# StarsX/RayTracedGGX

Measured on AMD Instinct MI355X. Metric: Mrays/s + ms/frame, bunny 1920x1080 1spp+denoise, 1/2/4/8 GPUs, higher is better.
Workload: dtype f32; 1 GPU; configs[1]: bunny.obj + rnl_cross env, 1920x1080, 1spp GGX reflection + full denoise chain (refl H,V; diff H,V, shared-memory variant; temporal; tone map), all-metal default materials, dt=1/60; parallelism=row strips x1, history_apron_rows=18, history_overreach_rows=0, setup_priming_frames=256, trace_workgroup_waves=12

## Files before the change

include/rtggx.h:

```cpp
#ifndef RTGGX_H
#define RTGGX_H

#include <stddef.h>
#include <stdint.h>

#ifdef __cplusplus
extern "C" {
#endif

typedef struct rtggx_context rtggx_context;

enum { RTGGX_GROUND = 0, RTGGX_MODEL_OBJ = 1, RTGGX_NUM_MESH = 2 };

typedef struct RtggxCBGlobal {
  float    WorldViewProjs[2][16];
  float    WorldViewProjsPrev[2][16];
  float    Worlds[2][12];
  float    WorldITs0[12];
  float    WorldIT1[11];
  uint32_t FrameIndex;
} RtggxCBGlobal;
typedef struct RtggxRayGenConstants {
  float ProjToWorld[16];
  float EyePt[4];
// ... 61 lines not shown
int  rtggx_create(rtggx_context** out, uint32_t width, uint32_t height, int device);
void rtggx_destroy(rtggx_context* ctx);

int  rtggx_set_strip(rtggx_context* ctx, uint32_t row_begin, uint32_t row_end);

int  rtggx_set_history_apron(rtggx_context* ctx, uint32_t rows);
int  rtggx_history_overreach(rtggx_context* ctx, uint32_t* rows, int reset);

int  rtggx_set_stream(rtggx_context* ctx, void* hip_stream);
int  rtggx_get_stream(rtggx_context* ctx, void** hip_stream);
#define RTGGX_MAX_PEERS 16
#define RTGGX_IPC_HANDLE_BYTES 64
int  rtggx_set_history_peers(rtggx_context* ctx, uint32_t world, const uint32_t* bounds, void* const* tss0, void* const* tss1);
int  rtggx_history_ipc_export(rtggx_context* ctx, void* handles, size_t bytes);
int  rtggx_history_ipc_open(rtggx_context* ctx, const void* handles, size_t bytes, void** tss0, void** tss1);

int  rtggx_set_async_compute(rtggx_context* ctx, int enable);

int  rtggx_set_mesh(rtggx_context* ctx, uint32_t slot, const float* verts, uint32_t num_verts,
                    const uint32_t* indices, uint32_t num_indices);
int  rtggx_set_env(rtggx_context* ctx, int format, uint32_t size, uint32_t mips, const void* data, size_t bytes);
enum { RTGGX_ENV_EQUIRECT = 0, RTGGX_ENV_VCROSS = 1, RTGGX_ENV_HCROSS = 2 };
enum { RTGGX_PIXELS_RGBE8 = 0, RTGGX_PIXELS_RGB32F = 1 };
int  rtggx_set_env_image(rtggx_context* ctx, int layout, int pixels, uint32_t width, uint32_t height, const void* data, size_t bytes,
                         uint32_t cube_size);
int  rtggx_generate_env_mips(rtggx_context* ctx);
#define RTGGX_ENV_FILTER_MIN_SAMPLES 64u
#define RTGGX_ENV_FILTER_MAX_SAMPLES 4096u
int  rtggx_prefilter_env(rtggx_context* ctx, uint32_t samples);
int  rtggx_set_material(rtggx_context* ctx, uint32_t mesh, const float base_color[4], float roughness, float metallic);
int  rtggx_set_metallic(rtggx_context* ctx, uint32_t mesh, float metallic);
int  rtggx_set_sampler(rtggx_context* ctx, int vndf);
int  rtggx_set_ray_rate(rtggx_context* ctx, uint32_t pixels_per_ray);
#define RTGGX_MAX_RECURSION_DEPTH 4u
int  rtggx_set_max_recursion_depth(rtggx_context* ctx, uint32_t depth);
#define RTGGX_MAX_SAMPLES_PER_PIXEL 8u
int  rtggx_set_samples_per_pixel(rtggx_context* ctx, uint32_t samples);
#define RTGGX_MIN_SAMPLE_SET 256u
#define RTGGX_MAX_SAMPLE_SET 65536u
int  rtggx_set_sample_set(rtggx_context* ctx, uint32_t size);
int  rtggx_set_accumulation(rtggx_context* ctx, int enable);
int  rtggx_reset_accumulation(rtggx_context* ctx);
int  rtggx_accumulated_frames(rtggx_context* ctx, uint32_t* frames);
int  rtggx_present_accumulation(rtggx_context* ctx);

typedef struct RtggxScore {
  uint64_t index;
  uint32_t frame_index;
  uint32_t pad;
  uint64_t pixels, covered;
  uint64_t skipped_out, skipped_raw;
  double se_out_rgb, se_out_luma;
  double se_raw_rgb, se_raw_luma;
  double ref_rgb2, ref_luma2;
  double se_out_rgb_cov, se_raw_rgb_cov, ref_rgb2_cov;
} RtggxScore;
enum { RTGGX_SCORE_RING = 256 };
int  rtggx_set_reference(rtggx_context* ctx, const void* rgba16f, size_t bytes);
int  rtggx_reference_from_accumulation(rtggx_context* ctx);
int  rtggx_set_scoring(rtggx_context* ctx, int enable);
int  rtggx_read_scores(rtggx_context* ctx, RtggxScore* out, uint32_t capacity, uint32_t* count);

int  rtggx_set_sample_map(rtggx_context* ctx, const uint8_t* counts, uint32_t blocks_x, uint32_t blocks_y);
int  rtggx_read_sample_map(rtggx_context* ctx, uint8_t* counts, uint32_t capacity, uint32_t* blocks_x, uint32_t* blocks_y);

int  rtggx_build_as(rtggx_context* ctx);

int  rtggx_refit_as(rtggx_context* ctx, uint32_t slot, const float* verts, uint32_t num_verts);
int  rtggx_refit_as_device(rtggx_context* ctx, uint32_t slot, const float* device_verts, uint32_t num_verts, void* hip_stream);
int  rtggx_set_refit_policy(rtggx_context* ctx, float rebuild_ratio, uint32_t steps_per_frame);
int  rtggx_refit_stats(rtggx_context* ctx, uint32_t slot, float* cost_ratio, uint32_t* refits, uint32_t* rebuilds);

int  rtggx_update_frame(rtggx_context* ctx, const RtggxFrameConstants* constants);
int  rtggx_update_as(rtggx_context* ctx);
int  rtggx_transform_sh(rtggx_context* ctx);
int  rtggx_render_visibility(rtggx_context* ctx);
int  rtggx_ray_trace(rtggx_context* ctx);
int  rtggx_denoise(rtggx_context* ctx, int use_shared_mem);
int  rtggx_tone_map(rtggx_context* ctx);

int  rtggx_debug_fuse_tone_map(rtggx_context* ctx, int mode);
int  rtggx_debug_placement(rtggx_context* ctx, int force_small, uint32_t* key, uint32_t* where);
int  rtggx_debug_tile_words(rtggx_context* ctx, int enable);
int  rtggx_debug_static_sky(rtggx_context* ctx, int enable);
int  rtggx_debug_sky_runs(rtggx_context* ctx, uint32_t* runs, uint32_t capacity, uint32_t* tiles_x, uint32_t* tiles_y, uint32_t* threshold);
int  rtggx_debug_settled_sky(rtggx_context* ctx, int enable);
int  rtggx_debug_settled_words(rtggx_context* ctx, uint32_t* words0, uint32_t* words1, uint32_t capacity, uint32_t* blocks_x, uint32_t* blocks_y, uint32_t* epoch);
int  rtggx_debug_collapse_weights(rtggx_context* ctx, const float* set, float* get);
int  rtggx_debug_fence_wait(rtggx_context* ctx, double* us_total, uint32_t* waits, int reset);

int  rtggx_sync(rtggx_context* ctx);
int  rtggx_ray_count(rtggx_context* ctx, uint64_t* rays);
int  rtggx_ray_total(rtggx_context* ctx, uint64_t* rays, int reset);
int  rtggx_debug_counters(rtggx_context* ctx, uint32_t* out, uint32_t n, int reset);
int  rtggx_debug_trace_split(rtggx_context* ctx, uint32_t work_per_wave, uint32_t max_shift, int capacity, uint32_t* last_demand);
int  rtggx_debug_trace_residency(rtggx_context* ctx, uint32_t force_waves, uint32_t* waves, float* share);
int  rtggx_debug_environment(rtggx_context* ctx, const float* dirs3, const float* levels, uint32_t n, int level0_path, float* rgb3);
int  rtggx_get_timings(rtggx_context* ctx, RtggxTimings* out);
#define RTGGX_KERNEL_RING 4096
int  rtggx_enable_timing(rtggx_context* ctx, int mode);
int  rtggx_kernel_times(rtggx_context* ctx, float* ms, uint32_t capacity, uint32_t* count);

int  rtggx_debug_shader_clock(rtggx_context* ctx, double* mhz);

int  rtggx_copy_bandwidth(rtggx_context* ctx, size_t bytes, int iterations, double* gbytes_per_s);

int  rtggx_buffer_size(rtggx_context* ctx, int buffer_id, size_t* bytes);
int  rtggx_readback(rtggx_context* ctx, int buffer_id, void* dst, size_t bytes);
int  rtggx_buffer_ptr(rtggx_context* ctx, int buffer_id, void** device_ptr);
int  rtggx_upload(rtggx_context* ctx, int buffer_id, const void* src, size_t bytes);
int  rtggx_frame_parity(rtggx_context* ctx, uint32_t* parity);
int  rtggx_bvh_root(rtggx_context* ctx, uint32_t slot, int32_t* root);

int  rtggx_trace_rays(rtggx_context* ctx, const float* rays, uint32_t n, float* out);

int  rtggx_trace_occlusion(rtggx_context* ctx, const float* rays, uint32_t n, uint32_t* occluded);

int  rtggx_set_sun(rtggx_context* ctx, const float direction[3], const float irradiance[3]);

int  rtggx_set_sun_reflections(rtggx_context* ctx, int enable);

#define RTGGX_MAX_SUN_ANGLE_DEGREES 10.0f
int  rtggx_set_sun_angle(rtggx_context* ctx, float degrees);

typedef struct RtggxLight {
  float position[3];  float range;
  float intensity[3]; float radius;
  float axis[3];      float cos_outer;
  float cos_inner;    float pad[3];
} RtggxLight;
#define RTGGX_MAX_LIGHTS 8u
int  rtggx_set_lights(rtggx_context* ctx, const RtggxLight* lights, uint32_t count);

int  rtggx_set_light_reflections(rtggx_context* ctx, int enable);

int  rtggx_set_light_sampling(rtggx_context* ctx, int mode);

typedef struct RtggxSunEstimate {
  double cos2_cone, cos2_ring;
  double peak_luma, mean_luma;
  double weight_all, weight_cone, weight_ring;
  double ring_rgb[3];
  double background[3];
  double excess[3];
  double moment[3];
  float  background_half[3];
  float  direction[3], irradiance[3];
  uint32_t found, removed;
  uint32_t peak_face, peak_x, peak_y;
  uint32_t texels_cone, texels_ring, texels_lit;
  uint32_t pad;
} RtggxSunEstimate;
int  rtggx_sun_from_env(rtggx_context* ctx, float cone_degrees, float ring_degrees, float min_contrast, int remove, RtggxSunEstimate* out);

#ifdef __cplusplus
}
#endif
#endif
```

raytracedggx_amd/capi.py:

```python
import ctypes as C
import os

import numpy as np

_HERE = os.path.dirname(os.path.abspath(__file__))
LIB_PATH = os.path.join(_HERE, "librtggx.so")

BUF_VISIBILITY, BUF_DEPTH, BUF_NORMAL, BUF_ROUGH_METAL, BUF_VELOCITY, BUF_RT_REFL, BUF_RT_DIFF, BUF_TSS0, BUF_TSS1, \
    BUF_FLT_RFL, BUF_FLT_DFF, BUF_BACKBUFFER, BUF_SH_COEFFS, BUF_BVH_NODES0, BUF_BVH_TRIS0, BUF_BVH_NODES1, BUF_BVH_TRIS1, \
    BUF_TLAS, BUF_ENV, BUF_BVH4_NODES0, BUF_BVH4_NODES1, BUF_BIN_WORK, BUF_BVH4_TOP0, BUF_BVH4_TOP1, BUF_EXCHANGE_TOKENS, \
    BUF_ACC_REFL, BUF_ACC_DIFF, BUF_CONVERGED = range(28)
MAX_PEERS, IPC_HANDLE_BYTES = 16, 64
FORMAT_RGBA32F, FORMAT_RGBA16F, FORMAT_BC6H_UF16, FORMAT_BC6H_SF16 = 2, 10, 95, 96
ENV_EQUIRECT, ENV_VCROSS, ENV_HCROSS = 0, 1, 2
PIXELS_RGBE8, PIXELS_RGB32F = 0, 1
ENV_FILTER_MIN_SAMPLES, ENV_FILTER_MAX_SAMPLES = 64, 4096
MAX_SUN_ANGLE_DEGREES = 10.0
MAX_LIGHTS = 8

_BUF_DTYPE = {BUF_VISIBILITY: np.uint32, BUF_DEPTH: np.uint32, BUF_NORMAL: np.uint32, BUF_ROUGH_METAL: np.uint16,
              BUF_VELOCITY: np.uint32, BUF_RT_REFL: np.uint32, BUF_RT_DIFF: np.uint32, BUF_TSS0: np.uint64, BUF_TSS1: np.uint64,
              BUF_FLT_RFL: np.uint64, BUF_FLT_DFF: np.uint64, BUF_BACKBUFFER: np.uint32, BUF_SH_COEFFS: np.float32,
              BUF_BVH_NODES0: np.uint32, BUF_BVH_TRIS0: np.uint32, BUF_BVH_NODES1: np.uint32, BUF_BVH_TRIS1: np.uint32,
              BUF_TLAS: np.float32, BUF_ENV: np.uint16, BUF_BVH4_NODES0: np.uint32, BUF_BVH4_NODES1: np.uint32, BUF_BIN_WORK: np.uint32,
              BUF_BVH4_TOP0: np.uint32, BUF_BVH4_TOP1: np.uint32, BUF_EXCHANGE_TOKENS: np.uint32,
              BUF_ACC_REFL: np.float32, BUF_ACC_DIFF: np.float32, BUF_CONVERGED: np.uint64}

EXPORTS = ["rtggx_last_error", "rtggx_create", "rtggx_destroy", "rtggx_set_strip", "rtggx_set_stream", "rtggx_set_mesh",
           "rtggx_set_env", "rtggx_set_material", "rtggx_set_metallic", "rtggx_build_as", "rtggx_update_frame", "rtggx_update_as",
           "rtggx_transform_sh", "rtggx_render_visibility", "rtggx_ray_trace", "rtggx_denoise", "rtggx_tone_map", "rtggx_sync",
           "rtggx_ray_count", "rtggx_get_timings", "rtggx_enable_timing", "rtggx_buffer_size", "rtggx_readback", "rtggx_buffer_ptr",
           "rtggx_upload", "rtggx_frame_parity", "rtggx_bvh_root", "rtggx_trace_rays", "rtggx_ray_total", "rtggx_kernel_times", "rtggx_debug_counters", "rtggx_debug_trace_split", "rtggx_debug_trace_residency", "rtggx_get_stream", "rtggx_set_history_peers", "rtggx_history_ipc_export", "rtggx_history_ipc_open",
           "rtggx_set_async_compute", "rtggx_set_history_apron", "rtggx_history_overreach", "rtggx_copy_bandwidth", "rtggx_refit_as", "rtggx_refit_as_device", "rtggx_refit_stats", "rtggx_set_refit_policy", "rtggx_set_sampler", "rtggx_set_ray_rate", "rtggx_set_max_recursion_depth", "rtggx_set_samples_per_pixel", "rtggx_debug_fuse_tone_map", "rtggx_debug_placement", "rtggx_debug_tile_words", "rtggx_debug_static_sky", "rtggx_debug_settled_sky", "rtggx_debug_settled_words", "rtggx_debug_sky_runs", "rtggx_debug_collapse_weights", "rtggx_debug_fence_wait", "rtggx_debug_shader_clock", "rtggx_debug_environment",
           "rtggx_set_accumulation", "rtggx_reset_accumulation", "rtggx_accumulated_frames", "rtggx_present_accumulation", "rtggx_set_sample_set",
           "rtggx_set_reference", "rtggx_reference_from_accumulation", "rtggx_set_scoring", "rtggx_read_scores",
           "rtggx_set_env_image", "rtggx_generate_env_mips", "rtggx_prefilter_env",
           "rtggx_set_sample_map", "rtggx_read_sample_map", "rtggx_trace_occlusion", "rtggx_set_sun", "rtggx_set_sun_reflections",
           "rtggx_sun_from_env", "rtggx_set_sun_angle", "rtggx_set_lights", "rtggx_set_light_reflections", "rtggx_set_light_sampling"]
SCORE_RING = 256


class Timings(C.Structure):
    _fields_ = [(n, C.c_float) for n in ("update_as", "visibility", "ray_trace", "spatial_refl_h", "spatial_refl_v",
                                         "spatial_diff_h", "spatial_diff_v", "temporal", "tone_map", "frame", "ray_trace_kernel")]


class Score(C.Structure):
    _fields_ = [("index", C.c_uint64), ("frame_index", C.c_uint32), ("pad", C.c_uint32), ("pixels", C.c_uint64), ("covered", C.c_uint64),
                ("skipped_out", C.c_uint64), ("skipped_raw", C.c_uint64)] + \
               [(n, C.c_double) for n in ("se_out_rgb", "se_out_luma", "se_raw_rgb", "se_raw_luma", "ref_rgb2", "ref_luma2",
                                          "se_out_rgb_cov", "se_raw_rgb_cov", "ref_rgb2_cov")]

    def as_dict(self):
        return {n: getattr(self, n) for n, _ in self._fields_ if n != "pad"}


class SunEstimate(C.Structure):
    _fields_ = [(n, C.c_double) for n in ("cos2_cone", "cos2_ring", "peak_luma", "mean_luma", "weight_all", "weight_cone", "weight_ring")] + \
               [(n, C.c_double * 3) for n in ("ring_rgb", "background", "excess", "moment")] + \
               [(n, C.c_float * 3) for n in ("background_half", "direction", "irradiance")] + \
               [(n, C.c_uint32) for n in ("found", "removed", "peak_face", "peak_x", "peak_y", "texels_cone", "texels_ring", "texels_lit", "pad")]

    def as_dict(self):
        out = {"bytes": bytes(self)}
        for n, t in self._fields_:
            if n != "pad":
                v = getattr(self, n)
                out[n] = v if t in (C.c_double, C.c_uint32) else np.array(list(v), np.float64 if t == C.c_double * 3 else np.float32)
        return out


class Light(C.Structure):
    _fields_ = [("position", C.c_float * 3), ("range", C.c_float), ("intensity", C.c_float * 3), ("radius", C.c_float),
                ("axis", C.c_float * 3), ("cos_outer", C.c_float), ("cos_inner", C.c_float), ("pad", C.c_float * 3)]

    @classmethod
    def of(cls, position, intensity, range, radius=0.0, axis=(0.0, 0.0, 0.0), cos_outer=-1.0, cos_inner=1.0):
        return cls((C.c_float * 3)(*position), range, (C.c_float * 3)(*intensity), radius, (C.c_float * 3)(*axis), cos_outer, cos_inner)


_lib = None


def load():
    global _lib
    if _lib is not None:
        return _lib
    if not os.path.exists(LIB_PATH):
        raise ImportError("librtggx.so is not built: run `python -c 'import __graft_entry__ as g; g.build()'` "
                          "or `make -C raytracedggx_amd` (hipcc, gfx950). There is no CPU path.")
    L = C.CDLL(LIB_PATH)
    L.rtggx_last_error.restype = C.c_char_p
    vp = C.c_void_p
    L.rtggx_create.argtypes = [C.POINTER(vp), C.c_uint32, C.c_uint32, C.c_int]
    L.rtggx_destroy.argtypes = [vp]
    L.rtggx_destroy.restype = None
    L.rtggx_set_strip.argtypes = [vp, C.c_uint32, C.c_uint32]
    L.rtggx_set_stream.argtypes = [vp, vp]
    L.rtggx_set_async_compute.argtypes = [vp, C.c_int]
    L.rtggx_set_ray_rate.argtypes = [vp, C.c_uint32]
    L.rtggx_set_max_recursion_depth.argtypes = [vp, C.c_uint32]
    L.rtggx_set_samples_per_pixel.argtypes = [vp, C.c_uint32]
    L.rtggx_set_sample_set.argtypes = [vp, C.c_uint32]
    L.rtggx_set_accumulation.argtypes = [vp, C.c_int]
    L.rtggx_reset_accumulation.argtypes = [vp]
    L.rtggx_accumulated_frames.argtypes = [vp, C.POINTER(C.c_uint32)]
    L.rtggx_present_accumulation.argtypes = [vp]
    L.rtggx_set_reference.argtypes = [vp, vp, C.c_size_t]
    L.rtggx_reference_from_accumulation.argtypes = [vp]
    L.rtggx_set_scoring.argtypes = [vp, C.c_int]
    L.rtggx_read_scores.argtypes = [vp, C.POINTER(Score), C.c_uint32, C.POINTER(C.c_uint32)]
    L.rtggx_set_sample_map.argtypes = [vp, vp, C.c_uint32, C.c_uint32]
    L.rtggx_read_sample_map.argtypes = [vp, vp, C.c_uint32, C.POINTER(C.c_uint32), C.POINTER(C.c_uint32)]
    L.rtggx_set_history_apron.argtypes = [vp, C.c_uint32]
    L.rtggx_debug_shader_clock.argtypes = [vp, C.POINTER(C.c_double)]
    L.rtggx_refit_as.argtypes = [vp, C.c_uint32, vp, C.c_uint32]
# ... 41 lines not shown
    pass


def _p(a):
    return a.ctypes.data_as(C.c_void_p)


class Context:

    def __init__(self, width, height, device=0):
        self.L = load()
        self.W, self.H = int(width), int(height)
        h = C.c_void_p()
        self._check(self.L.rtggx_create(C.byref(h), self.W, self.H, int(device)))
        self.h = h

    def _check(self, rc):
        if rc != 0:
            raise RtggxError("librtggx: %s (code %d)" % (self.L.rtggx_last_error().decode(), rc))

    def close(self):
        if getattr(self, "h", None):
            self.L.rtggx_destroy(self.h)
            self.h = None

    def __del__(self):
        try:
            self.close()
        except Exception:
            pass

    def set_strip(self, row_begin, row_end):
        self._check(self.L.rtggx_set_strip(self.h, row_begin, row_end))

    def set_stream(self, stream_handle):
        self._check(self.L.rtggx_set_stream(self.h, C.c_void_p(stream_handle)))

    def shader_clock_mhz(self):
        m = C.c_double()
        self._check(self.L.rtggx_debug_shader_clock(self.h, C.byref(m)))
        return m.value

    def copy_bandwidth(self, nbytes=1 << 30, iterations=8):
        g = C.c_double()
        self._check(self.L.rtggx_copy_bandwidth(self.h, int(nbytes), int(iterations), C.byref(g)))
        return g.value

    def set_history_apron(self, rows):
        self._check(self.L.rtggx_set_history_apron(self.h, int(rows)))

    def history_overreach(self, reset=True):
        n = C.c_uint32()
        self._check(self.L.rtggx_history_overreach(self.h, C.byref(n), int(reset)))
        return n.value

    def set_async_compute(self, enable):
        self._check(self.L.rtggx_set_async_compute(self.h, int(bool(enable))))

    def set_mesh(self, slot, verts, indices):
        v = np.ascontiguousarray(verts, np.float32).reshape(-1, 6)
        i = np.ascontiguousarray(indices, np.uint32).reshape(-1)
        self._check(self.L.rtggx_set_mesh(self.h, slot, _p(v), v.shape[0], _p(i), i.size))

    def refit_as(self, slot, verts):
        v = np.ascontiguousarray(verts, np.float32).reshape(-1, 6)
        self._check(self.L.rtggx_refit_as(self.h, slot, _p(v), v.shape[0]))

    def refit_as_device(self, slot, device_ptr, num_verts, stream=0):
        self.L.rtggx_refit_as_device.argtypes = [C.c_void_p, C.c_uint32, C.c_void_p, C.c_uint32, C.c_void_p]
        self._check(self.L.rtggx_refit_as_device(self.h, slot, C.c_void_p(int(device_ptr)), int(num_verts), C.c_void_p(int(stream) or None)))

    def fence_wait(self, reset=True):
        us, n = C.c_double(0.0), C.c_uint32(0)
        self.L.rtggx_debug_fence_wait.argtypes = [C.c_void_p, C.POINTER(C.c_double), C.POINTER(C.c_uint32), C.c_int]
        self._check(self.L.rtggx_debug_fence_wait(self.h, C.byref(us), C.byref(n), 1 if reset else 0))
        return us.value, n.value

    def fuse_tone_map(self, mode):
        self._check(self.L.rtggx_debug_fuse_tone_map(self.h, -1 if mode is None else 1 if mode else 0))

    def tile_words(self, enable):
        self._check(self.L.rtggx_debug_tile_words(self.h, 1 if enable else 0))

    def static_sky(self, enable):
        self._check(self.L.rtggx_debug_static_sky(self.h, 1 if enable else 0))

    def sky_runs(self):
        tiles = ((self.W + 15) // 16) * ((self.H + 15) // 16 + 1)
        runs = np.zeros(tiles, np.uint32)
        tx, ty, th = C.c_uint32(), C.c_uint32(), C.c_uint32()
        self.L.rtggx_debug_sky_runs.argtypes = [C.c_void_p, C.c_void_p, C.c_uint32, C.c_void_p, C.c_void_p, C.c_void_p]
        self._check(self.L.rtggx_debug_sky_runs(self.h, _p(runs), tiles, C.byref(tx), C.byref(ty), C.byref(th)))
        return runs[:tx.value * ty.value].reshape(ty.value, tx.value), int(th.value)

    def settled_sky(self, enable):
        self.L.rtggx_debug_settled_sky.argtypes = [C.c_void_p, C.c_int]
        self._check(self.L.rtggx_debug_settled_sky(self.h, 1 if enable else 0))

    def settled_words(self):
        n = ((self.W + 63) // 64) * ((self.H + 3) // 4)
        w = np.zeros((2, n), np.uint32)
        bx, by, ep = C.c_uint32(), C.c_uint32(), C.c_uint32()
        self.L.rtggx_debug_settled_words.argtypes = [C.c_void_p, C.c_void_p, C.c_void_p, C.c_uint32, C.c_void_p, C.c_void_p, C.c_void_p]
        self._check(self.L.rtggx_debug_settled_words(self.h, _p(w[0]), _p(w[1]), n, C.byref(bx), C.byref(by), C.byref(ep)))
        return np.ascontiguousarray(w.reshape(2, bx.value, by.value).transpose(0, 2, 1)), int(ep.value)

    def placement(self, force_small=-1):
        k, w = C.c_uint32(), C.c_uint32()
        self.L.rtggx_debug_placement.argtypes = [C.c_void_p, C.c_int, C.c_void_p, C.c_void_p]
        self._check(self.L.rtggx_debug_placement(self.h, int(force_small), C.byref(k), C.byref(w)))
        names = ("main", "B", "C", "R", "?")
        key = {n: bool((k.value >> i) & 1) for i, n in enumerate(("small", "strip", "deforming", "diffuse", "caller_stream"))}
        where = {"raster": names[(w.value >> 16) & 15], "gen": names[w.value & 15], "trace": names[(w.value >> 4) & 15], "shade": names[(w.value >> 8) & 15], "frames_in_flight": (w.value >> 12) & 15}
        return key, where

    def collapse_weights(self, area=None, tris=None):
        self.L.rtggx_debug_collapse_weights.argtypes = [C.c_void_p, C.c_void_p, C.c_void_p]
        get = (C.c_float * 2)()
        if area is not None:
            st = (C.c_float * 2)(float(area), float(tris))
            self._check(self.L.rtggx_debug_collapse_weights(self.h, st, get))
        else:
            self._check(self.L.rtggx_debug_collapse_weights(self.h, None, get))
        return float(get[0]), float(get[1])

    def set_history_peers(self, bounds, tss0, tss1):
        self.L.rtggx_set_history_peers.argtypes = [C.c_void_p, C.c_uint32, C.c_void_p, C.c_void_p, C.c_void_p]
        if bounds is None:
            self._check(self.L.rtggx_set_history_peers(self.h, 0, None, None, None))
            return
        world = len(bounds) - 1
        b = (C.c_uint32 * (world + 1))(*[int(x) for x in bounds])
        p0 = (C.c_void_p * world)(*[C.c_void_p(int(x) or None) for x in tss0])
        p1 = (C.c_void_p * world)(*[C.c_void_p(int(x) or None) for x in tss1])
        self._check(self.L.rtggx_set_history_peers(self.h, world, b, p0, p1))

    def history_ipc_export(self):
        self.L.rtggx_history_ipc_export.argtypes = [C.c_void_p, C.c_void_p, C.c_size_t]
        buf = C.create_string_buffer(2 * IPC_HANDLE_BYTES)
        self._check(self.L.rtggx_history_ipc_export(self.h, buf, len(buf.raw)))
        return bytes(buf.raw)

    def history_ipc_open(self, handles):
        self.L.rtggx_history_ipc_open.argtypes = [C.c_void_p, C.c_char_p, C.c_size_t, C.c_void_p, C.c_void_p]
        p0, p1 = C.c_void_p(), C.c_void_p()
        self._check(self.L.rtggx_history_ipc_open(self.h, bytes(handles), len(handles), C.byref(p0), C.byref(p1)))
        return int(p0.value), int(p1.value)

    def set_sampler(self, vndf):
        self._check(self.L.rtggx_set_sampler(self.h, 1 if vndf else 0))

    def set_ray_rate(self, pixels_per_ray):
        self._check(self.L.rtggx_set_ray_rate(self.h, int(pixels_per_ray)))

    def set_max_recursion_depth(self, depth):
        self._check(self.L.rtggx_set_max_recursion_depth(self.h, int(depth)))

    def set_samples_per_pixel(self, samples):
        self._check(self.L.rtggx_set_samples_per_pixel(self.h, int(samples)))

    def set_sample_set(self, size):
        self._check(self.L.rtggx_set_sample_set(self.h, int(size)))

    def set_accumulation(self, enable):
        self._check(self.L.rtggx_set_accumulation(self.h, 1 if enable else 0))

# ... 261 lines not shown
```

raytracedggx_amd/csrc/debug.hip:

```cpp
#include <cstring>
#include "capi_internal.h"
#include "rt_queue.h"
namespace rt {
__global__ void __launch_bounds__(256) copyKernel(const float4* __restrict__ src, float4* __restrict__ dst, size_t n) {
  for (size_t i = (size_t)blockIdx.x * 256u + threadIdx.x; i < n; i += (size_t)gridDim.x * 256u) dst[i] = src[i];
}
typedef float __attribute__((ext_vector_type(4))) CopyVec4;
__global__ void __launch_bounds__(256) copyKernelNT(const CopyVec4* __restrict__ src, CopyVec4* __restrict__ dst, size_t n) {
  for (size_t i = (size_t)blockIdx.x * 256u + threadIdx.x; i < n; i += (size_t)gridDim.x * 256u) __builtin_nontemporal_store(__builtin_nontemporal_load(&src[i]), &dst[i]);
}
}
using namespace rt;

extern "C" {
int rtggx_ray_count(rtggx_context* c, uint64_t* rays) {
  RT_CHECK_CTX(c);
  uint32_t h[256];
  RT_HIP(syncStreams(c));
  RT_HIP(hipMemcpy(h, c->lastRayCounter32, sizeof h, hipMemcpyDeviceToHost));
  uint64_t s = 0; for (auto v : h) s += v;
  *rays = s;
  return 0;
}

int rtggx_debug_counters(rtggx_context* c, uint32_t* out, uint32_t n, int reset) {
  RT_CHECK_CTX(c);
  if (n > 768) { setError("rtggx_debug_counters: at most 768 words"); return -1; }
  RT_HIP(syncStreams(c));
  RT_HIP(hipMemcpy(out, c->rayCounterBuf + 1024, (size_t)n * 4, hipMemcpyDeviceToHost));
  if (reset) { RT_HIP(hipMemset(c->rayCounterBuf + 1024, 0, 768 * 4)); RT_HIP(hipStreamSynchronize(nullptr)); }
  return 0;
}

int rtggx_debug_fence_wait(rtggx_context* c, double* usTotal, uint32_t* waits, int reset) {
  RT_CHECK_CTX(c);
  if (usTotal) *usTotal = c->fenceWaitUs;
  if (waits) *waits = c->fenceWaits;
  if (reset) { c->fenceWaitUs = 0.0; c->fenceWaits = 0u; }
  return 0;
}
int rtggx_debug_fuse_tone_map(rtggx_context* c, int mode) {
  RT_CHECK_CTX(c);
  c->fuseToneMap = mode < 0 ? -1 : mode != 0;
  return 0;
}
int rtggx_debug_tile_words(rtggx_context* c, int enable) {
  RT_CHECK_CTX(c);
  c->useTileWords = enable != 0;
  c->sky.breakRuns(SkyBreak::TileWordsSwitch);
  return 0;
}
int rtggx_debug_static_sky(rtggx_context* c, int enable) {
  RT_CHECK_CTX(c);
  c->sky.enableStaticSky(enable != 0);
  return 0;
}
int rtggx_debug_sky_runs(rtggx_context* c, uint32_t* runs, uint32_t capacity, uint32_t* tilesX, uint32_t* tilesY, uint32_t* threshold) {
  RT_CHECK_CTX(c);
  const uint32_t n = c->sky.genTilesX() * c->sky.genTilesY();
  if (!runs || capacity < n || n > c->skyTiles) { setError("rtggx_debug_sky_runs: room for %u words", n); return -1; }
  RT_HIP(syncStreams(c));
  if (n) RT_HIP(hipMemcpy(runs, c->cur().skyRun, (size_t)n * 4, hipMemcpyDeviceToHost));
  for (uint32_t i = 0; i < n; ++i) runs[i] = (runs[i] >> 8) == c->sky.epoch() ? runs[i] & 0xFFu : 0u;
  if (tilesX) *tilesX = c->sky.genTilesX();
  if (tilesY) *tilesY = c->sky.genTilesY();
  if (threshold) *threshold = RT_SKY_PREV_RUN + 1u;
  return 0;
}
int rtggx_debug_settled_sky(rtggx_context* c, int enable) {
  RT_CHECK_CTX(c);
  c->sky.enableSettledSky(enable != 0);
  return 0;
}
int rtggx_debug_settled_words(rtggx_context* c, uint32_t* words0, uint32_t* words1, uint32_t capacity, uint32_t* blocksX, uint32_t* blocksY, uint32_t* epoch) {
  RT_CHECK_CTX(c);
  const uint32_t n = c->settledX * c->settledY;
  if (!words0 || !words1 || capacity < n) { setError("rtggx_debug_settled_words: room for %u words each", n); return -1; }
  RT_HIP(syncStreams(c));
  uint32_t* const out[2] = {words0, words1};
  for (int p = 0; p < 2 && n; ++p)
    RT_HIP(hipMemcpy2D(out[p], (size_t)c->settledY * 4, c->settled[p] + c->settledPitch + 1u, (size_t)c->settledPitch * 4, (size_t)c->settledY * 4, c->settledX, hipMemcpyDeviceToHost));
  if (blocksX) *blocksX = c->settledX;
  if (blocksY) *blocksY = c->settledY;
  if (epoch) *epoch = c->sky.epoch();
  return 0;
}
int rtggx_debug_placement(rtggx_context* c, int forceSmall, uint32_t* key, uint32_t* where) {
  RT_CHECK_CTX(c);
  if (forceSmall < -1 || forceSmall > 1) { setError("rtggx_debug_placement: force_small is -1, 0 or 1"); return -1; }
  c->forcePlacement = forceSmall;
  if (forceSmall >= 0) c->lastTraceSmall = forceSmall == 1;
  if (key) *key = c->lastPlacement[0];
  if (where) *where = c->lastPlacement[1];
  return 0;
}
int rtggx_debug_collapse_weights(rtggx_context* c, const float* set, float* get) {
  RT_CHECK_CTX(c);
  if (set) { if (!(set[0] >= 0.0f) || !(set[1] >= 0.0f) || !(set[0] + set[1] > 0.0f)) { setError("rtggx_debug_collapse_weights: two non-negative weights, not both zero"); return -1; }
             c->collapseWeights[0] = set[0]; c->collapseWeights[1] = set[1]; }
  if (get) { get[0] = c->collapseWeights[0]; get[1] = c->collapseWeights[1]; }
  return 0;
}
int rtggx_debug_trace_residency(rtggx_context* c, uint32_t forceWaves, uint32_t* waves, float* share) {
  RT_CHECK_CTX(c);
  if (forceWaves != 0u && forceWaves != 10u && forceWaves != 12u && forceWaves != 14u && forceWaves != 16u) { setError("rtggx_debug_trace_residency: %u waves: 0, 10, 12, 14 or 16", forceWaves); return -1; }
  c->traceWavesForced = forceWaves;
  if (forceWaves) c->traceWaves = forceWaves;
  if (waves) *waves = c->traceWaves;
  if (share) *share = c->traceShare;
  return 0;
}

int rtggx_debug_environment(rtggx_context* c, const float* dirs3, const float* levels, uint32_t n, int level0Path, float* rgb3) {
  RT_CHECK_CTX(c);
  if (!c->env.texels) { setError("rtggx_debug_environment: no environment map"); return -1; }
  if (n == 0 || !dirs3 || !rgb3 || (!levels && !level0Path)) { setError("rtggx_debug_environment: no directions, levels or result (n %u)", n); return -1; }
  DevBuf<float> dD, dL, dO;
  hipError_t e = alloc(dD, (size_t)n * 3);
  if (e == hipSuccess) e = alloc(dO, (size_t)n * 3);
  if (e == hipSuccess && levels) e = alloc(dL, (size_t)n);
  if (e == hipSuccess) e = hipMemcpy(dD, dirs3, (size_t)n * 12, hipMemcpyHostToDevice);
  if (e == hipSuccess && levels) e = hipMemcpy(dL, levels, (size_t)n * 4, hipMemcpyHostToDevice);
  int r = 0;
  if (e == hipSuccess) r = launchDebugEnvironment(c, dD, dL, n, level0Path, dO, c->streamMain);
  if (e == hipSuccess && !r) e = hipStreamSynchronize(c->streamMain);
  if (e == hipSuccess && !r) e = hipMemcpy(rgb3, dO, (size_t)n * 12, hipMemcpyDeviceToHost);
  if (e != hipSuccess) { setError("rtggx_debug_environment: %s", hipGetErrorString(e)); return -2; }
  return r;
}

int rtggx_debug_trace_split(rtggx_context* c, uint32_t workPerWave, uint32_t maxShift, int capacity, uint32_t* lastDemand) {
  RT_CHECK_CTX(c);
// ... 245 lines not shown
```

raytracedggx_amd/csrc/denoise.hip:

```cpp
#include <cstring>
#include <type_traits>
#include "rtggx_context.h"

namespace rt {

#define RT_RADIUS 16
#ifndef RT_VBW
#define RT_VBW 16
#define RT_VBH 16
#endif

RT_DEV float rcpFast(float x) { return __builtin_amdgcn_rcpf(x); }

struct GTexel { float nx, ny, nz, nw, rough, metal, depth; };

RT_DEV GTexel loadG(const uint32_t* __restrict__ normal, const uint16_t* __restrict__ roughMetal, const uint32_t* __restrict__ depth32,
                    int x, int y, int W, int H) {
  GTexel g;
  if (x < 0 || y < 0 || x >= W || y >= H) { g.nx = g.ny = g.nz = -1023.0f; g.nw = 0.0f; g.rough = 0.0f; g.metal = 0.0f; g.depth = 0.0f; return g; }
  const size_t i = (size_t)y * W + x;
  const uint32_t n = normal[i];
  g.nx = (float)(2 * (int)(n & 1023u) - 1023);
  g.ny = (float)(2 * (int)((n >> 10) & 1023u) - 1023);
  g.nz = (float)(2 * (int)((n >> 20) & 1023u) - 1023);
// ... 35 lines not shown
RT_DEV uint32_t skyRunMin6(const uint32_t* words, uint32_t epoch, uint32_t i0, uint32_t i1, uint32_t i2, uint32_t i3, uint32_t i4, uint32_t i5) {
  uint32_t w[6];
  asm volatile("s_load_dword %0, %6, %7\n\ts_load_dword %1, %6, %8\n\ts_load_dword %2, %6, %9\n\ts_load_dword %3, %6, %10\n\ts_load_dword %4, %6, %11\n\ts_load_dword %5, %6, %12\n\ts_waitcnt lgkmcnt(0)"
               : "=&s"(w[0]), "=&s"(w[1]), "=&s"(w[2]), "=&s"(w[3]), "=&s"(w[4]), "=&s"(w[5])
               : "s"(words), "s"(RT_SGPR(i0 * 4u)), "s"(RT_SGPR(i1 * 4u)), "s"(RT_SGPR(i2 * 4u)), "s"(RT_SGPR(i3 * 4u)), "s"(RT_SGPR(i4 * 4u)), "s"(RT_SGPR(i5 * 4u)) : "memory");
  uint32_t run = 0xFFu;
#pragma unroll
  for (int k = 0; k < 6; ++k) run = min(run, (w[k] >> 8) == epoch ? w[k] & 0xFFu : 0u);
  return run;
}

typedef uint32_t U2 __attribute__((ext_vector_type(2)));
typedef uint32_t U4 __attribute__((ext_vector_type(4)));
RT_DEV void loadTemporalWords(const uint32_t* rowA, const uint32_t* rowB, const uint32_t* col0, const uint32_t* col1, const uint32_t* col2,
                              U4& a4, U2& a2, U4& b4, U2& b2, U4& c0, U4& c1, U4& c2) {
  asm volatile("s_load_dwordx4 %0, %7, 0x0\n\ts_load_dwordx2 %1, %7, 0x10\n\ts_load_dwordx4 %2, %8, 0x0\n\ts_load_dwordx2 %3, %8, 0x10\n\t"
               "s_load_dwordx4 %4, %9, 0x0\n\ts_load_dwordx4 %5, %10, 0x0\n\ts_load_dwordx4 %6, %11, 0x0\n\ts_waitcnt lgkmcnt(0)"
               : "=&s"(a4), "=&s"(a2), "=&s"(b4), "=&s"(b2), "=&s"(c0), "=&s"(c1), "=&s"(c2)
               : "s"(rowA), "s"(rowB), "s"(col0), "s"(col1), "s"(col2) : "memory");
}
RT_DEV void loadToneMapWords(const uint32_t* col0, const uint32_t* col1, const uint32_t* col2, U4& a4, U2& a2, U4& b4, U2& b2, U4& c4, U2& c2) {
  asm volatile("s_load_dwordx4 %0, %6, 0x0\n\ts_load_dwordx2 %1, %6, 0x10\n\ts_load_dwordx4 %2, %7, 0x0\n\ts_load_dwordx2 %3, %7, 0x10\n\t"
               "s_load_dwordx4 %4, %8, 0x0\n\ts_load_dwordx2 %5, %8, 0x10\n\ts_waitcnt lgkmcnt(0)"
               : "=&s"(a4), "=&s"(a2), "=&s"(b4), "=&s"(b2), "=&s"(c4), "=&s"(c2) : "s"(col0), "s"(col1), "s"(col2) : "memory");
}

#define RT_LOG2E 1.44269504088896341f

struct Centre { float nx, ny, nz, depth, rough, gaussK , depthK ; };
#define RT_NORMAL_SCALE_SQ 1046529.0f
RT_DEV float log2OfDot(float I) {
  const float d = fmaxf((I - RT_NORMAL_SCALE_SQ) * (1.0f / RT_NORMAL_SCALE_SQ), -1.0f);
  const float xr = 1.0f + d;
  const float dropped = (1.0f - xr) + d;
  return __builtin_fmaf(dropped, RT_LOG2E, __builtin_amdgcn_logf(xr));
}
template <bool DIFFUSE, int UNIFORM = 0>
RT_DEV float tapWeight(const Centre& c, int i, float nx, float ny, float nz, float depth, float rough) {
#pragma clang fp contract(fast)
  const float I = __builtin_fmaf(c.nz, nz, __builtin_fmaf(c.ny, ny, c.nx * nx));
  const float lg = log2OfDot(I);
  const float dd = fabsf(c.depth - depth) * c.depthK;
  if (DIFFUSE) return __builtin_amdgcn_exp2f(__builtin_fmaf(32.0f, lg, -dd));
  const float pw = 512.0f * lg;
  const float e = __builtin_fmaf(c.gaussK, (float)(i * i), -dd);
  const float w = __builtin_amdgcn_exp2f(pw >= 128.0f ? pw : pw + e);
  if (UNIFORM == 2) return w;
  const float flag = (__float_as_uint(rough) >> 31) ? 0.0f : 1.0f;
  if (UNIFORM == 1) return w * flag;
  const float t = saturatef(fabsf(fabsf(rough) - c.rough) * 2.0f);
  return (w * (1.0f - t * t * (3.0f - 2.0f * t))) * flag;
}
template <bool DIFFUSE>
RT_DEV Centre makeCentre(float nx, float ny, float nz, float depth, float rough, int W, int H) {
  Centre c; c.nx = nx; c.ny = ny; c.nz = nz; c.depth = depth; c.rough = rough;
  const int br = DIFFUSE ? 0 : (int)clampf(0.1f * rough * (float)W, 0.0f, (float)H * 0.05f);
  const float sigma = (float)(br + 1) * (1.0f / 3.0f);
  c.gaussK = (-0.5f * RT_LOG2E) * rcpFast(sigma * sigma);
  c.depthK = depth * (4.0f * RT_LOG2E);
  return c;
}
template <int MODE>
RT_DEV void storeFiltered(const Targets& T, size_t pix, float mx, float my, float mz, float wsum) {
  const float rw = rcpFast(wsum);
  f3 mu = mk3(mx * rw, my * rw, mz * rw);
  if (MODE == 0 || MODE == 2) T.scratch[pix] = packRGBA16F(mu.x, mu.y, mu.z, 0.0f);
  if (MODE == 1) { mu = ITM3(mu); const uint2 v = packRGBA16F(mu.x, mu.y, mu.z, 1.0f); if (T.fltRfl) T.fltRfl[pix] = v; T.fltDff[pix] = v; }
  if (MODE == 3) {
    const f4 dest = unpackRGBA16F(T.fltRfl[pix]);
    mu = ITM3(mu);
    T.fltDff[pix] = packRGBA16F(dest.x + mu.x, dest.y + mu.y, dest.z + mu.z, dest.w);
  }
}
template <int MODE>
RT_DEV void storeSkipped(const Targets& T, size_t pix) {
  if (MODE == 1) { const f3 s = unpackR11G11B10F(T.rtRefl[pix]); const uint2 v = packRGBA16F(s.x, s.y, s.z, 0.0f); if (T.fltRfl) T.fltRfl[pix] = v; T.fltDff[pix] = v; }
}
template <int MODE>
RT_DEV f3 tapColour(const Targets& T, size_t ti) {
  if (MODE & 1) { const f4 v = unpackRGBA16F(T.scratch[ti]); return mk3(v.x, v.y, v.z); }
  return TM3(unpackR11G11B10F(MODE >= 2 ? T.rtDiff[ti] : T.rtRefl[ti]));
}

template <int MODE>
__global__ void __launch_bounds__(256) spatialDirectKernel(Targets T) {
  constexpr bool vertical = (MODE & 1) != 0;
  constexpr bool diffuse = MODE >= 2;
  const int x = blockIdx.x * 64 + (threadIdx.x & 63);
  const int y = T.rowBegin + blockIdx.y * 4 + (threadIdx.x >> 6);
  if (x >= T.W || y >= T.rowEnd) return;
  const size_t pix = (size_t)y * T.W + x;
  const GTexel gc = loadG(T.normal, T.roughMetal, T.depth32, x, y, T.W, T.H);
  if (diffuse ? (gc.nw <= 0.0f || gc.metal >= 1.0f) : (gc.nw <= 0.0f)) { storeSkipped<MODE>(T, pix); return; }
  const Centre c = makeCentre<diffuse>(gc.nx, gc.ny, gc.nz, gc.depth, gc.rough, T.W, T.H);
  float mx = 0.0f, my = 0.0f, mz = 0.0f, wsum = 0.0f;
  for (int i = -RT_RADIUS; i <= RT_RADIUS; ++i) {
    const int tx = vertical ? x : x + i, ty = vertical ? y + i : y;
    const bool inside = tx >= 0 && ty >= 0 && tx < T.W && ty < T.H;
    const GTexel g = loadG(T.normal, T.roughMetal, T.depth32, tx, ty, T.W, T.H);
    if (diffuse && (g.nw <= 0.0f || g.metal >= 1.0f)) continue;
    const f3 src = inside ? tapColour<MODE>(T, (size_t)ty * T.W + tx) : mk3(0.0f, 0.0f, 0.0f);
    const float w = tapWeight<diffuse>(c, i, g.nx, g.ny, g.nz, g.depth, g.nw > 0.0f ? g.rough : __uint_as_float(__float_as_uint(g.rough) | 0x80000000u));
    mx = __builtin_fmaf(src.x, w, mx); my = __builtin_fmaf(src.y, w, my); mz = __builtin_fmaf(src.z, w, mz);
    wsum += w;
  }
  storeFiltered<MODE>(T, pix, mx, my, mz, wsum);
}

typedef float V4 __attribute__((ext_vector_type(4)));
template <int MODE>
__global__ void __launch_bounds__(256) spatialTiledKernel(Targets T) {
  constexpr bool vertical = (MODE & 1) != 0;
  constexpr bool diffuse = MODE >= 2;
  constexpr int BW = vertical ? RT_VBW : 64, BH = vertical ? RT_VBH : 4;
  constexpr int TW = vertical ? RT_VBW : 96, TH = vertical ? RT_VBH + 2 * RT_RADIUS : 4;
  constexpr int PER = vertical ? BW * BH / 256 : 1, ROWSTEP = 256 / BW;
  constexpr int N = TW * TH;
  __shared__ V4 smA[N], smB[N];
  __shared__ uint32_t roughLo, roughHi, unflagged;
  if (threadIdx.x == 0) { roughLo = 0xFFFFFFFFu; roughHi = 0u; unflagged = 0u; }
  const int bx0 = blockIdx.x * BW, by0 = T.rowBegin + blockIdx.y * BH;
  const int lx = threadIdx.x % BW, ly = threadIdx.x / BW;
  const int x = bx0 + lx;

  static_assert(RT_VBW <= 32 && RT_VBH <= 32, "the V block spans at most two tiles across and three down");
  bool nothingDrawn;
  { const uint32_t txLast = (uint32_t)T.tilesX - 1u, tx0 = (uint32_t)bx0 >> 4, tx1 = min(tx0 + 1u, txLast);
    const uint32_t ty0 = (uint32_t)(by0 - T.tileRow0) >> 4, ty1 = (uint32_t)(min(by0 + BH, T.rowEnd) - 1 - T.tileRow0) >> 4;
    const uint32_t r0 = ty0 * (uint32_t)T.tilesX, r1 = ty1 * (uint32_t)T.tilesX, rm = ((ty0 + ty1) >> 1) * (uint32_t)T.tilesX;
    if (MODE == 1 && T.skyRun != nullptr && skyRunMin6(T.skyRun, T.skyEpoch, r0 + tx0, r0 + tx1, rm + tx0, rm + tx1, r1 + tx0, r1 + tx1) >= RT_SKY_V_RUN) return;
    nothingDrawn = vertical ? tileWordsOr6(T.tileWords, r0 + tx0, r0 + tx1, rm + tx0, rm + tx1, r1 + tx0, r1 + tx1) == 0u
                            : tileWordsOr(T.tileWords, r0 + tx0, r0 + tx1, r0 + min(tx0 + 2u, txLast), r0 + min(tx0 + 3u, txLast)) == 0u; }
  if (nothingDrawn) {
    if (MODE == 1) {
#pragma unroll
      for (int k = 0; k < PER; ++k) { const int y = by0 + ly + k * ROWSTEP; if (x < T.W && y < T.rowEnd) storeSkipped<MODE>(T, (size_t)y * T.W + x); }
    }
    return;
  }
  bool todo[PER]; bool any = false;
#pragma unroll
  for (int k = 0; k < PER; ++k) {
    const int y = by0 + ly + k * ROWSTEP;
    todo[k] = false;
    if (x < T.W && y < T.rowEnd) {
      const size_t pix = (size_t)y * T.W + x;
      const bool skip = (T.normal[pix] >> 30) == 0u || (diffuse && (T.roughMetal[pix] >> 8) == 255u);
      if (skip) storeSkipped<MODE>(T, pix); else { todo[k] = true; any = true; }
    }
  }
  if (!__syncthreads_or(any ? 1 : 0)) return;

  const int ox = vertical ? bx0 : bx0 - RT_RADIUS, oy = vertical ? by0 - RT_RADIUS : by0;
  uint32_t myLo = 0xFFFFFFFFu, myHi = 0u, myUnflagged = 0u;
  for (int t = threadIdx.x; t < N; t += 256) {
    const int tx = ox + t % TW, ty = oy + t / TW;
    float v[8] = {0.0f, 0.0f, 0.0f, 0.0f, 0.0f, 0.0f, 0.0f, 0.0f};
    const bool inside = tx >= 0 && ty >= 0 && tx < T.W && ty < T.H;
    const GTexel g = loadG(T.normal, T.roughMetal, T.depth32, tx, ty, T.W, T.H);
    v[3] = g.depth; v[4] = g.rough;
    if (diffuse) {
      if (g.nw > 0.0f && g.metal < 1.0f) {
        const f3 src = tapColour<MODE>(T, (size_t)ty * T.W + tx);
        v[0] = g.nx; v[1] = g.ny; v[2] = g.nz; v[5] = src.x; v[6] = src.y; v[7] = src.z;
      }
    } else {
      v[0] = g.nx; v[1] = g.ny; v[2] = g.nz;
      if (g.nw <= 0.0f) { v[4] = __uint_as_float(__float_as_uint(g.rough) | 0x80000000u); myUnflagged = 1u; }
      else { myLo = min(myLo, __float_as_uint(g.rough)); myHi = max(myHi, __float_as_uint(g.rough)); }
      if (inside) { const f3 src = tapColour<MODE>(T, (size_t)ty * T.W + tx); v[5] = src.x; v[6] = src.y; v[7] = src.z; }
    }
    smA[t] = V4{v[0], v[1], v[2], v[3]}; smB[t] = V4{v[4], v[5], v[6], v[7]};
  }
  if (!diffuse) {
    for (int o = 32; o > 0; o >>= 1) { myLo = min(myLo, (uint32_t)__shfl_down((int)myLo, o)); myHi = max(myHi, (uint32_t)__shfl_down((int)myHi, o)); }
    const unsigned long long anyUnflagged = __ballot(myUnflagged != 0u);
    if ((threadIdx.x & 63) == 0) { atomicMin(&roughLo, myLo); atomicMax(&roughHi, myHi); if (anyUnflagged) atomicOr(&unflagged, 1u); }
  }
  __syncthreads();
  const int uniform = diffuse ? 0 : (roughLo != roughHi ? 0 : unflagged ? 1 : 2);

  auto filter = [&](auto uniformTag) {
    constexpr int UNIFORM = decltype(uniformTag)::value;
#pragma unroll
    for (int k = 0; k < PER; ++k) {
      if (!todo[k]) continue;
      const int y = by0 + ly + k * ROWSTEP;
      const int ci = vertical ? (ly + k * ROWSTEP + RT_RADIUS) * TW + lx : ly * TW + lx + RT_RADIUS;
      const V4 ca = smA[ci];
      const Centre c = makeCentre<diffuse>(ca.x, ca.y, ca.z, ca.w, smB[ci].x, T.W, T.H);
      float mx = 0.0f, my = 0.0f, mz = 0.0f, wsum = 0.0f;
      typedef __attribute__((address_space(3))) const V4 LdsV4;
      LdsV4* pa = (LdsV4*)&smA[ci - RT_RADIUS * (vertical ? TW : 1)]; LdsV4* pb = (LdsV4*)&smB[ci - RT_RADIUS * (vertical ? TW : 1)];
      asm volatile("" : "+v"(pa)); asm volatile("" : "+v"(pb));
#pragma unroll
      for (int i = -RT_RADIUS; i <= RT_RADIUS; ++i) {
        const int ti = (i + RT_RADIUS) * (vertical ? TW : 1);
        const V4 a = pa[ti], b = pb[ti];
        const float w = tapWeight<diffuse, UNIFORM>(c, i, a.x, a.y, a.z, a.w, b.x);
        mx = __builtin_fmaf(b.y, w, mx); my = __builtin_fmaf(b.z, w, my); mz = __builtin_fmaf(b.w, w, mz);
        wsum += w;
      }
      storeFiltered<MODE>(T, (size_t)y * T.W + x, mx, my, mz, wsum);
    }
// ... 296 lines not shown
  if (WORDS && T.settledIn != nullptr) {
    static_assert(RT_TM_ROWS == 4 * RT_TP_ROWS, "a tone-map block is four blocks of the temporal pass high");
    const uint32_t* col = T.settledIn + blockIdx.x * T.settledPitch + blockIdx.y * 4u;
    U4 a4, b4, c4; U2 a2, b2, c2;
    loadToneMapWords(col, col + T.settledPitch, col + 2u * T.settledPitch, a4, a2, b4, b2, c4, c2);
    const uint32_t w[18] = {a4.x, a4.y, a4.z, a4.w, a2.x, a2.y, b4.x, b4.y, b4.z, b4.w, b2.x, b2.y, c4.x, c4.y, c4.z, c4.w, c2.x, c2.y};
    bool skip = true;
#pragma unroll
    for (int k = 0; k < 18; ++k) skip = skip & settledWord(w[k], T.skyEpoch);
    if (skip) return;
  }
  {
    const int ox = blockIdx.x * 64 - 1, oy = T.rowBegin + blockIdx.y * RT_TM_ROWS - 1;
    constexpr int N = (RT_TM_ROWS + 2) * 66, PER = (N + 255) / 256;
    f4 c[PER];
#pragma unroll
    for (int k = 0; k < PER; ++k) { const int t = threadIdx.x + 256 * k; c[k] = t < N ? loadRGBA16(T.scratch, ox + t % 66, oy + t / 66, W, H) : f4{0.0f, 0.0f, 0.0f, 0.0f}; }
#pragma unroll
    for (int k = 0; k < PER; ++k) {
      const int t = threadIdx.x + 256 * k;
      if (t < N) tile[t / 66][t % 66] = make_float4(c[k].x * rcpFast(c[k].x + 0.5f), c[k].y * rcpFast(c[k].y + 0.5f), c[k].z * rcpFast(c[k].z + 0.5f), c[k].w);
    }
  }
  __syncthreads();
  const int lx = (threadIdx.x & 63) + 1;
  const int x = blockIdx.x * 64 + (threadIdx.x & 63);
  if (x >= T.W) return;
#pragma unroll
  for (int k = 0; k < RT_TM_ROWS / 4; ++k) {
    const int ly = (threadIdx.x >> 6) + 4 * k + 1;
    const int y = T.rowBegin + blockIdx.y * RT_TM_ROWS + (threadIdx.x >> 6) + 4 * k;
    if (y >= T.rowEnd) continue;
    const float4 c0 = tile[ly][lx], c1 = tile[ly][lx - 1], c2 = tile[ly][lx + 1], c3 = tile[ly - 1][lx], c4 = tile[ly + 1][lx];
    float lx_ = -4.0f * c0.x, ly_ = -4.0f * c0.y, lz_ = -4.0f * c0.z;
    lx_ += c1.x; ly_ += c1.y; lz_ += c1.z;
    lx_ += c2.x; ly_ += c2.y; lz_ += c2.z;
    lx_ += c3.x; ly_ += c3.y; lz_ += c3.z;
    lx_ += c4.x; ly_ += c4.y; lz_ += c4.z;
    T.backbuffer[(size_t)y * W + x] = packRGBA8(c0.x - 0.2f * lx_, c0.y - 0.2f * ly_, c0.z - 0.2f * lz_, c0.w);
  }
}

static Targets makeTargets(rtggx_context* c, const FrameParams& fp, RowPass pass) {
  Targets T;
  const InputSet& set = c->cur();
  T.normal = set.normal; T.roughMetal = set.roughMetal; T.depth32 = set.depth32; T.velocity = set.velocity;
  T.rtRefl = set.rtRefl; T.rtDiff = set.rtDiff;
  T.scratch = c->tss[c->frameParity]; T.history = c->tss[c->frameParity ^ 1u]; T.fltRfl = c->fltRfl; T.fltDff = c->fltDff; T.backbuffer = c->backbuffer;
  T.W = (int)fp.W; T.H = (int)fp.H;
  uint32_t rb, re; passRows(fp, pass, rb, re);
  T.rowBegin = (int)rb; T.rowEnd = (int)re;
  passRows(fp, ROWS_FINAL, rb, re);
  T.outBegin = (int)rb; T.outEnd = (int)re;
  const bool strip = fp.rowBegin > 0u || fp.rowEnd < fp.H;
  T.histLo = (int)(fp.rowBegin > c->historyApron ? fp.rowBegin - c->historyApron : 0u);
  T.histHi = (int)(fp.rowEnd + c->historyApron < fp.H ? fp.rowEnd + c->historyApron : fp.H);
  T.histReach = strip ? c->histReach : nullptr;
  const bool peers = strip && c->peerWorld > 1u && c->dPeerTable != nullptr;
  T.peerHist = peers ? reinterpret_cast<const uint2* const*>(c->dPeerTable.get()) + (c->frameParity ^ 1u) * RT_MAX_PEERS : nullptr;
  T.peerBounds = peers ? reinterpret_cast<const uint32_t*>(reinterpret_cast<const uint2* const*>(c->dPeerTable.get()) + 2 * RT_MAX_PEERS) : nullptr;
  T.peerWorld = peers ? (int)c->peerWorld : 0;
  { uint32_t gb, ge; passRows(fp, ROWS_GBUFFER, gb, ge);
    T.tileWords = c->tileWords(gb, ge); T.tilesX = (int)((fp.W + 15) / 16); T.tileRow0 = (int)gb; }
  T.skyRun = nullptr; T.skyEpoch = 0u;
  T.settledOut = nullptr; T.settledIn = nullptr; T.settledPitch = c->settledPitch;
  return T;
}

static bool wholeFrame(const rtggx_context* c, const FrameParams& fp) { return fp.rowBegin == 0u && fp.rowEnd == fp.H && fp.W == c->W && fp.H == c->H; }

int launchDenoise(rtggx_context* c, const FrameParams& fp, int useLds, hipStream_t s, hipEvent_t done, bool fuseToneMap) {
  c->frameParity ^= 1u;
  if (fp.rowEnd <= fp.rowBegin) return 0;
  const Targets TH = makeTargets(c, fp, ROWS_GBUFFER), TV = makeTargets(c, fp, ROWS_VFILTER), TT = makeTargets(c, fp, ROWS_TEMPORAL);
  const dim3 block(256);
  auto grid = [&](const Targets& T, uint32_t bw, uint32_t bh) { return dim3((fp.W + bw - 1) / bw, (T.rowEnd - T.rowBegin + bh - 1) / bh); };
  auto mark = [&](int i) { if (c->timing) hipEventRecord(c->tev[i], s); };
  const bool anyDiffuse = fp.mat.RoughMetals[0][1] < 1.0f || fp.mat.RoughMetals[1][1] < 1.0f;
  c->fltRflIsFltDff = !anyDiffuse;
  Targets TVr = TV; if (!anyDiffuse) TVr.fltRfl = nullptr;
  { SkyChain::VFacts now;
    now.frame = c->frameCounter; now.gbufferRow0 = (uint32_t)TV.tileRow0; now.rows[0] = (uint32_t)TV.rowBegin; now.rows[1] = (uint32_t)TV.rowEnd; now.fltRflNull = TVr.fltRfl == nullptr;
    if (c->sky.reflectionV(now) && useLds) { TVr.skyRun = c->cur().skyRun; TVr.skyEpoch = c->sky.epoch(); } }
  if (useLds) {
    hipLaunchKernelGGL(spatialTiledKernel<0>, grid(TH, 64, 4), block, 0, s, TH); mark(4);
    hipLaunchKernelGGL(spatialTiledKernel<1>, grid(TV, RT_VBW, RT_VBH), block, 0, s, TVr); mark(5);
    if (anyDiffuse) hipLaunchKernelGGL(spatialTiledKernel<2>, grid(TH, 64, 4), block, 0, s, TH);
    mark(6);
    if (anyDiffuse) hipLaunchKernelGGL(spatialTiledKernel<3>, grid(TV, RT_VBW, RT_VBH), block, 0, s, TV);
    mark(7);
  } else if (!anyDiffuse) {
    hipLaunchKernelGGL(spatialDirectKernel<0>, grid(TH, 64, 4), block, 0, s, TH); mark(4);
    hipLaunchKernelGGL(spatialDirectKernel<1>, grid(TV, 64, 4), block, 0, s, TVr); mark(5); mark(6); mark(7);
  } else {
    hipLaunchKernelGGL(spatialDirectKernel<0>, grid(TH, 64, 4), block, 0, s, TH); mark(4);
    hipLaunchKernelGGL(spatialDirectKernel<1>, grid(TV, 64, 4), block, 0, s, TV); mark(5);
    hipLaunchKernelGGL(spatialDirectKernel<2>, grid(TH, 64, 4), block, 0, s, TH); mark(6);
    hipLaunchKernelGGL(spatialDirectKernel<3>, grid(TV, 64, 4), block, 0, s, TV); mark(7);
  }
  Targets TTs = TT;
  { SkyChain::TemporalFacts now;
    now.frame = c->frameCounter; now.gbufferRow0 = (uint32_t)TT.tileRow0; now.rows[0] = (uint32_t)TT.rowBegin; now.rows[1] = (uint32_t)TT.rowEnd;
    now.parity = c->frameParity; now.width = fp.W; now.fused = fuseToneMap; now.whole = wholeFrame(c, fp);
    const SkyChain::TemporalDecision d = c->sky.temporal(now);
    if (d.keepsWords) { TTs.settledOut = c->settled[c->frameParity]; TTs.skyEpoch = c->sky.epoch(); }
    if (d.maySkip) { TTs.settledIn = c->settled[c->frameParity ^ 1u]; TTs.skyRun = c->cur().skyRun; } }
  if (fuseToneMap) {
    const dim3 g((fp.W + RT_TT_W - 1) / RT_TT_W, (uint32_t)(TT.outEnd - TT.outBegin + RT_TT_H - 1) / RT_TT_H), b(RT_TT_TW * RT_TT_TH);
    launch(temporalToneKernel, g, b, s, nullptr, done, TT);
    c->sky.backBufferWrittenElsewhere();
  } else launch(TTs.settledOut ? temporalKernel<true> : temporalKernel<false>, grid(TT, 64, RT_TP_ROWS), block, s, nullptr, done, TTs);
  mark(8);
  RT_HIP(hipGetLastError());
  return 0;
}

int launchToneMap(rtggx_context* c, const FrameParams& fp, hipStream_t s, hipEvent_t done, const uint2* source) {
  if (fp.rowEnd <= fp.rowBegin) return 0;
  Targets T = makeTargets(c, fp, ROWS_FINAL);
  if (source) T.scratch = const_cast<uint2*>(source);
  { SkyChain::ToneMapFacts now;
    now.frame = c->frameCounter; now.rows[0] = (uint32_t)T.rowBegin; now.rows[1] = (uint32_t)T.rowEnd; now.parity = c->frameParity; now.fromTss = source == nullptr; now.whole = wholeFrame(c, fp);
    if (c->sky.toneMap(now)) { T.settledIn = c->settled[c->frameParity]; T.skyEpoch = c->sky.epoch(); } }
  const dim3 grid((fp.W + 63) / 64, (uint32_t)(T.rowEnd - T.rowBegin + RT_TM_ROWS - 1) / RT_TM_ROWS), block(256);
  launch(T.settledIn ? toneMapKernel<true> : toneMapKernel<false>, grid, block, s, nullptr, done, T);
  RT_HIP(hipGetLastError());
  return 0;
}

}
```

raytracedggx_amd/csrc/frame.hip:

```cpp
#include <cstring>
#include <chrono>
#include "capi_internal.h"
#include "rt_queue.h"
namespace rt {
static void invert4x4(const float* a , float* out) {
  double m[16], inv[16];
  for (int i = 0; i < 16; ++i) m[i] = (double)a[i];
  inv[0] = m[5] * m[10] * m[15] - m[5] * m[11] * m[14] - m[9] * m[6] * m[15] + m[9] * m[7] * m[14] + m[13] * m[6] * m[11] - m[13] * m[7] * m[10];
  inv[4] = -m[4] * m[10] * m[15] + m[4] * m[11] * m[14] + m[8] * m[6] * m[15] - m[8] * m[7] * m[14] - m[12] * m[6] * m[11] + m[12] * m[7] * m[10];
  inv[8] = m[4] * m[9] * m[15] - m[4] * m[11] * m[13] - m[8] * m[5] * m[15] + m[8] * m[7] * m[13] + m[12] * m[5] * m[11] - m[12] * m[7] * m[9];
  inv[12] = -m[4] * m[9] * m[14] + m[4] * m[10] * m[13] + m[8] * m[5] * m[14] - m[8] * m[6] * m[13] - m[12] * m[5] * m[10] + m[12] * m[6] * m[9];
  inv[1] = -m[1] * m[10] * m[15] + m[1] * m[11] * m[14] + m[9] * m[2] * m[15] - m[9] * m[3] * m[14] - m[13] * m[2] * m[11] + m[13] * m[3] * m[10];
  inv[5] = m[0] * m[10] * m[15] - m[0] * m[11] * m[14] - m[8] * m[2] * m[15] + m[8] * m[3] * m[14] + m[12] * m[2] * m[11] - m[12] * m[3] * m[10];
  inv[9] = -m[0] * m[9] * m[15] + m[0] * m[11] * m[13] + m[8] * m[1] * m[15] - m[8] * m[3] * m[13] - m[12] * m[1] * m[11] + m[12] * m[3] * m[9];
  inv[13] = m[0] * m[9] * m[14] - m[0] * m[10] * m[13] - m[8] * m[1] * m[14] + m[8] * m[2] * m[13] + m[12] * m[1] * m[10] - m[12] * m[2] * m[9];
  inv[2] = m[1] * m[6] * m[15] - m[1] * m[7] * m[14] - m[5] * m[2] * m[15] + m[5] * m[3] * m[14] + m[13] * m[2] * m[7] - m[13] * m[3] * m[6];
  inv[6] = -m[0] * m[6] * m[15] + m[0] * m[7] * m[14] + m[4] * m[2] * m[15] - m[4] * m[3] * m[14] - m[12] * m[2] * m[7] + m[12] * m[3] * m[6];
  inv[10] = m[0] * m[5] * m[15] - m[0] * m[7] * m[13] - m[4] * m[1] * m[15] + m[4] * m[3] * m[13] + m[12] * m[1] * m[7] - m[12] * m[3] * m[5];
  inv[14] = -m[0] * m[5] * m[14] + m[0] * m[6] * m[13] + m[4] * m[1] * m[14] - m[4] * m[2] * m[13] - m[12] * m[1] * m[6] + m[12] * m[2] * m[5];
  inv[3] = -m[1] * m[6] * m[11] + m[1] * m[7] * m[10] + m[5] * m[2] * m[11] - m[5] * m[3] * m[10] - m[9] * m[2] * m[7] + m[9] * m[3] * m[6];
  inv[7] = m[0] * m[6] * m[11] - m[0] * m[7] * m[10] - m[4] * m[2] * m[11] + m[4] * m[3] * m[10] + m[8] * m[2] * m[7] - m[8] * m[3] * m[6];
  inv[11] = -m[0] * m[5] * m[11] + m[0] * m[7] * m[9] + m[4] * m[1] * m[11] - m[4] * m[3] * m[9] - m[8] * m[1] * m[7] + m[8] * m[3] * m[5];
  inv[15] = m[0] * m[5] * m[10] - m[0] * m[6] * m[9] - m[4] * m[1] * m[10] + m[4] * m[2] * m[9] + m[8] * m[1] * m[6] - m[8] * m[2] * m[5];
  const double det = m[0] * inv[0] + m[1] * inv[4] + m[2] * inv[8] + m[3] * inv[12];
// ... 73 lines not shown

int rtggx_transform_sh(rtggx_context* c) {
  RT_CHECK_CTX(c);
  return projectSH(c, c->streamAS);
}

struct Placement {
  bool small, strip, deforming, diffuse, callerStream;
  hipStream_t raster, gen, trace, shade;
  uint32_t framesInFlight;
  bool alternate, shadeWithTrace;
};
static Placement placeFrame(const rtggx_context* c, const FrameParams& fp, uint32_t frame) {
  Placement P;
  P.small = c->lastTraceSmall;
  P.strip = fp.rowBegin > 0u || fp.rowEnd < fp.H;
  P.deforming = c->mesh[0].deforming || c->mesh[1].deforming;
  P.diffuse = fp.mat.RoughMetals[0][1] < 1.0f || fp.mat.RoughMetals[1][1] < 1.0f;
  P.callerStream = c->externalStream;
  const bool async = c->asyncCompute && c->streamVis != nullptr;
  P.gen = async ? c->streamVis : c->streamMain;
  P.raster = P.gen;
  P.alternate = async && c->streamRefit != nullptr && P.small && !P.deforming && (frame & 1u) != 0u;
  P.trace = !async ? c->streamMain : P.alternate ? c->streamRefit : c->streamAS;
  P.shadeWithTrace = async && !c->timing && P.small && !P.deforming;
  P.shade = P.shadeWithTrace ? P.trace : c->streamMain;
  P.framesInFlight = async && !P.small && (P.deforming || P.diffuse) ? RT_SETS - 1u : RT_SETS;
  return P;
}

static int waitForSet(rtggx_context* c, const InputSet& set) {
  if (set.readRecorded && hipEventQuery(set.evRead) != hipSuccess) {
    const auto t0 = std::chrono::steady_clock::now();
    RT_HIP(hipEventSynchronize(set.evRead));
    c->fenceWaitUs += std::chrono::duration<double, std::micro>(std::chrono::steady_clock::now() - t0).count(); ++c->fenceWaits;
  }
  return 0;
}

int rtggx_render_visibility(rtggx_context* c) {
  RT_CHECK_CTX(c);
  if (!c->haveConstants) { setError("rtggx_render_visibility: no frame constants"); return -1; }
  if (!c->shDone && c->env.texels) { const int r = projectSH(c, c->streamAS); if (r) return r; }
  settleSetRead(c);
  ++c->frameCounter;
  c->maxDepth = c->depthRequested; c->samples = c->samplesRequested; c->accumulate = c->accumulateRequested; c->sun = c->sunRequested; c->sunAngle = c->sunAngleRequested; c->sunReflections = c->sunReflectionsRequested; c->lights = c->lightsRequested; c->lightReflections = c->lightReflectionsRequested; c->lightSampling = c->lightSamplingRequested;
  c->scoring = c->scoringRequested && c->reference != nullptr;
  c->sampleMap = c->sampleMapRequested;
  bool resendConstants = false;
  if (c->sampleSet != c->sampleSetRequested) {
    if (c->slotRendered) RT_HIP(syncStreams(c));
    c->sampleSet = c->sampleSetRequested;
    c->slots[c->slot].sampleMask = c->sampleSet - 1u;
    resendConstants = c->slotUploaded;
  }
  c->denoiseIssued = false; c->toneMapDone = false;
  c->selectSet(c->setAhead(1u));
  { const int r = waitForSet(c, c->cur()); if (r) return r; }
  const Placement P = placeFrame(c, c->slots[c->slot], c->frameCounter);
  if (P.framesInFlight < RT_SETS) { const int r = waitForSet(c, c->sets[c->setAhead(RT_SETS - P.framesInFlight)]); if (r) return r; }
  c->refitIssued = false;
  { const int r = issuePendingRefits(c, &c->refitIssued); if (r) return r; }
  const hipStream_t s = P.raster;
  if (c->evVisStream && c->evVisStream != s) RT_HIP(hipStreamWaitEvent(s, c->evVis, 0));
  { const FrameEvents& g = c->frameEvents(c->frameCounter + 2u);
    if (c->frameCounter >= 2u && g.genFrame == c->frameCounter - 2u && g.genStream != s) RT_HIP(hipStreamWaitEvent(s, g.gen, 0)); }
  if (c->slotUploaded && s != c->streamAS) RT_HIP(hipStreamWaitEvent(s, c->evAS, 0));
  if (c->refitIssued && c->asyncCompute && s != c->streamRefit) RT_HIP(hipStreamWaitEvent(s, c->evRefit, 0));
  if (c->timing) hipEventRecord(c->tev[2], s);
  int r = launchVisibility(c, c->slots[c->slot], s, c->streamVis ? c->evVis : nullptr);
  c->slotRendered = true;
  if (resendConstants) c->slotUploaded = false;
  if (c->streamVis) c->evVisStream = s;
  if (c->timing) hipEventRecord(c->tev[13], s);
  if (!r) r = issueRebuildSteps(c);
  return r;
}

int rtggx_ray_trace(rtggx_context* c) {
  RT_CHECK_CTX(c);
  if (!c->haveConstants || !c->asBuilt) { setError("rtggx_ray_trace: %s", c->asBuilt ? "no frame constants" : "rtggx_build_as has not been called"); return -1; }
  if (!c->env.texels) { setError("rtggx_ray_trace: no environment map"); return -1; }
  { const int r = ensureParams(c); if (r) return r; }
  const uint32_t f = c->frameCounter;
  const FrameParams& fp = c->slots[c->slot];
  const Placement P = placeFrame(c, fp, f);
  c->lastPlacement[0] = P.small | (P.strip << 1) | (P.deforming << 2) | (P.diffuse << 3) | (P.callerStream << 4);
  const auto streamId = [&](hipStream_t st) { return st == c->streamMain ? 0u : st == c->streamAS ? 1u : st == c->streamVis ? 2u : st == c->streamRefit ? 3u : 4u; };
  c->lastPlacement[1] = streamId(P.gen) | (streamId(P.trace) << 4) | (streamId(P.shade) << 8) | (P.framesInFlight << 12) | (streamId(P.raster) << 16);
  const hipStream_t sGen = P.gen;
  if (c->evVisStream && c->evVisStream != sGen) RT_HIP(hipStreamWaitEvent(sGen, c->evVis, 0));
  const hipStream_t sTrace = P.trace;
  c->traceSpillHalf = P.alternate ? 1u : 0u;
  if (sGen != sTrace) {
    if (c->frameEvents(f + 2u).traceRecorded) RT_HIP(hipStreamWaitEvent(sGen, c->frameEvents(f + 2u).trace, 0));
    if (c->slotUploaded) RT_HIP(hipStreamWaitEvent(sGen, c->evAS, 0));
  }
  if (c->refitIssued && c->asyncCompute) RT_HIP(hipStreamWaitEvent(sTrace, c->evRefit, 0));
  if (c->timing) hipEventRecord(c->tev[3], sGen);
  FrameEvents& ev = c->frameEvents(f);
  const bool shadeWithTrace = P.shadeWithTrace && sGen != sTrace && sTrace != c->streamMain;
  if (c->shadeWroteDiff && !P.diffuse && !c->lastFrameDiffuse && c->diffStream) {
    if (c->diffStream != sGen) { RT_HIP(hipEventRecord(c->evRT, c->diffStream)); RT_HIP(hipStreamWaitEvent(sGen, c->evRT, 0)); }
    c->shadeWroteDiff = false;
  }
  c->lastFrameDiffuse = P.diffuse;
  c->genCarriesDiff = !c->shadeWroteDiff;
  int r = launchRayTrace(c, fp, sGen, sTrace, shadeWithTrace ? nullptr : ev.trace);
  ev.traceRecorded = true;
  c->lastRayCounter32 = c->rayCounter32;
  c->shadeWroteDiff = !c->genCarriesDiff || P.diffuse;
  if (shadeWithTrace) {
    if (!c->genCarriesDiff && c->shadeStream && c->shadeStream != sTrace) {
      if (c->shadeStream == c->streamMain) { RT_HIP(hipEventRecord(c->evRT, c->streamMain)); RT_HIP(hipStreamWaitEvent(sTrace, c->evRT, 0)); }
      else if (c->frameEvents(f + 3u).traceRecorded) RT_HIP(hipStreamWaitEvent(sTrace, c->frameEvents(f + 3u).trace, 0));
    }
    if (!r) r = launchShade(c, fp, sTrace, ev.trace);
    c->shadeStream = sTrace;
    RT_HIP(hipStreamWaitEvent(c->streamMain, ev.trace, 0));
  } else {
    RT_HIP(hipStreamWaitEvent(c->streamMain, ev.trace, 0));
    if (!r) r = launchShade(c, fp, c->streamMain);
    c->shadeStream = c->streamMain;
  }
  c->diffStream = c->shadeStream;
  if (c->rayRate == 4u) {
    if (!r) r = launchReconstruct(c, fp, c->streamMain);
    c->diffStream = c->streamMain;
  }
  if (c->sun.on) {
    if (!r) r = launchSun(c, fp, c->streamMain);
    c->shadeStream = c->diffStream = c->streamMain;
  }
  if (c->lights.count) {
    if (!r) r = launchLights(c, fp, c->streamMain);
    c->shadeStream = c->diffStream = c->streamMain;
  }
  if (c->accumulate) {
    if (!r) r = launchAccumulate(c, fp, c->streamMain);
    if (!r) ++c->accumFrames;
  }
  c->setReadDeferred = (int)c->setIndex;
  if (c->timing) hipEventRecord(c->tev[14], c->streamMain);
  return r;
}

int rtggx_denoise(rtggx_context* c, int useSharedMem) {
  RT_CHECK_CTX(c);
  if (!c->haveConstants) { setError("rtggx_denoise: no frame constants"); return -1; }
  if (c->timing) hipEventRecord(c->tev[9], c->streamMain);
  const bool fuse = !c->timing && !c->scoring && (c->fuseToneMap > 0 || (c->fuseToneMap < 0 && c->lastTraceSmall));
  const int r = launchDenoise(c, c->slots[c->slot], useSharedMem, c->streamMain, fuse ? c->cur().evRead : nullptr, fuse);
  if (fuse) { c->cur().readRecorded = true; c->setReadDeferred = -1; } else c->setReadDeferred = (int)c->setIndex;
  if (!r && c->scoring && c->reference) { const int rs = launchScore(c, c->slots[c->slot], c->streamMain); if (rs) return rs; }
  c->denoiseIssued = true; c->toneMapDone = fuse && c->slots[c->slot].rowEnd > c->slots[c->slot].rowBegin;
  return r;
}

int rtggx_tone_map(rtggx_context* c) {
  RT_CHECK_CTX(c);
  if (!c->haveConstants) { setError("rtggx_tone_map: no frame constants"); return -1; }
  int r = 0;
  if (c->toneMapDone) c->toneMapDone = false;
  else {
    const bool carry = c->setReadDeferred >= 0;
    r = launchToneMap(c, c->slots[c->slot], c->streamMain, carry ? c->sets[c->setReadDeferred].evRead : nullptr);
// ... 15 lines not shown
```

raytracedggx_amd/csrc/raytrace.hip:

```cpp
#include <cstring>
#include <type_traits>
#include "rt_queue.h"
#include "rt_traverse.h"
#include "rt_surface.h"

namespace rt {


struct EnvRef { const uint2* __restrict__ texels; uint32_t size, mips; const uint32_t* __restrict__ mipOffset; };

RT_DEV void cubeFaceUV(f3 d, int& face, float& u, float& v) {
  const float ax = fabsf(d.x), ay = fabsf(d.y), az = fabsf(d.z);
  if (ax >= ay && ax >= az) { face = d.x >= 0.0f ? 0 : 1; u = (d.x >= 0.0f ? -d.z : d.z) / ax; v = -d.y / ax; }
  else if (ay >= az) { face = d.y >= 0.0f ? 2 : 3; u = d.x / ay; v = (d.y >= 0.0f ? d.z : -d.z) / ay; }
  else { face = d.z >= 0.0f ? 4 : 5; u = (d.z >= 0.0f ? d.x : -d.x) / az; v = -d.y / az; }
}
RT_DEV f3 cubeFaceDir(int face, float u, float v) {
  switch (face) {
    case 0: return mk3(1.0f, -v, -u);
    case 1: return mk3(-1.0f, -v, u);
    case 2: return mk3(u, 1.0f, v);
    case 3: return mk3(u, -1.0f, -v);
    case 4: return mk3(u, -v, 1.0f);
    default: return mk3(-u, -v, -1.0f);
// ... 284 lines not shown
          const f3 f0 = mk3(lerpf(0.04f, color.x, rghMtl.y), lerpf(0.04f, color.y, rghMtl.y), lerpf(0.04f, color.z, rghMtl.y));
          const float NoV = saturatef(dot3(N, V));
          const float VoH = saturatef(dot3(V, Hh));
          const f3 F = fSchlick(f0, VoH);
          const float vis = visSmith(rghMtl.x, NoV, NoL);
          const float NoH = saturatef(dot3(N, Hh));
          const float k = 4.0f * VoH / NoH;
          wantRefl = true;
          rr.ox = P.x; rr.oy = P.y; rr.oz = P.z;
          rr.dx = R.x; rr.dy = R.y; rr.dz = R.z;
          rr.pixel = (uint32_t)pix; rr.skip = skip; rr.flags = 0u;
          rr.wx = ((NoL * F.x) * vis) * k; rr.wy = ((NoL * F.y) * vis) * k; rr.wz = ((NoL * F.z) * vis) * k;
          if (vndf) {
            const float a2 = a * a;
            const float g1l = (2.0f * NoL) / (NoL + sqrtf(NoL * (NoL - NoL * a2) + a2));
            rr.wx = F.x * g1l; rr.wy = F.y * g1l; rr.wz = F.z * g1l;
          }
        }
      }
      if (rghMtl.y < 1.0f) {
        if (traced) {
          const float cosTheta = 1.0f - 2.0f * xiY;
          const float sinTheta = sqrtf(1.0f - cosTheta * cosTheta);
          const f3 dir = normalize3(N + mk3(cosPhi * sinTheta, sinPhi * sinTheta, cosTheta));
          wantDiff = true;
          rd.ox = P.x; rd.oy = P.y; rd.oz = P.z;
          rd.dx = dir.x; rd.dy = dir.y; rd.dz = dir.z;
          rd.pixel = (uint32_t)pix; rd.skip = skip; rd.flags = 1u;
          rd.wx = color.x * (1.0f - 0.04f); rd.wy = color.y * (1.0f - 0.04f); rd.wz = color.z * (1.0f - 0.04f);
        }
      } else if (A.diffPrev != nullptr) A.diffOut[pix] = A.diffPrev[pix];
    }
  }
  if (threadIdx.x == 0) { A.skyOut[tile] = skyWordOut; if (clearNext) A.visDirtyNextOut[tile] = 0u; }
  if constexpr (RATE == 4) { rayGenQuadBin(A, wantRefl, wantDiff, rr, rd); return; }

  const uint32_t bin = blockIdx.x * 4u + wave;
  const unsigned long long maskR = __ballot(wantRefl), maskD = __ballot(wantDiff), below = (1ull << lane) - 1ull;
  const uint32_t nR = (uint32_t)__popcll(maskR);
  RayRec* dst = A.rays + (size_t)bin * A.binSlots;
  HitKey* keys = A.hits + (size_t)bin * A.binSlots;
  if (wantRefl) { const uint32_t k = (uint32_t)__popcll(maskR & below); dst[k] = rr; keys[k] = hitKey(RT_RAY_TMAX, 0xFFFFFFFFu); }
  const uint32_t kD = nR + (uint32_t)__popcll(maskD & below);
  if (wantDiff && kD < A.binSlots) { dst[kD] = rd; keys[kD] = hitKey(RT_RAY_TMAX, 0xFFFFFFFFu); }
  const uint32_t nRaysInBin = min(nR + (uint32_t)__popcll(maskD), A.binSlots);
  if (A.binWork == nullptr) {
    if (lane == 0) A.binCount[bin] = nRaysInBin;
    return;
  }
  __shared__ uint32_t want[4], listBase;
  uint32_t shift = 0u, n = 0u;
  if (lane == 0) {
    const uint32_t w = A.binWork[bin];
    A.binWork[bin] = 0u;
    while (shift < A.splitMaxShift && (w >> shift) > A.splitWork) ++shift;
    n = (shift || w > A.frontWork) ? 1u << shift : 0u;
    want[wave] = n;
  }
  __syncthreads();
  if (threadIdx.x == 0) { const uint32_t total = want[0] + want[1] + want[2] + want[3]; listBase = total ? atomicAdd(A.splitCount, total) : 0u; }
  __syncthreads();
  if (lane == 0) {
    uint32_t base = listBase, mark = 0u;
    for (uint32_t k = 0; k < wave; ++k) base += want[k];
    if (n) {
      const bool fits = base + n <= A.splitCap;
      for (uint32_t k = 0; k < n && base + k < A.splitCap; ++k) A.splitList[base + k] = fits ? ((shift << 28) | (k << 24) | bin) : 0xFFFFFFFFu;
      mark = fits ? (shift << 1) | 1u : 0u;
    }
    A.binCount[bin] = nRaysInBin | (mark << 8);
  }
}

struct ShadeArgs {
  const RayRec* rays; const HitKey* hits; const uint32_t* binCount; uint32_t binSlots;
  const float4* fat0; const float4* fat1;
  const uint2* env; const uint32_t* envMipOffset; uint32_t envSize, envMips;
  const float* sh;
  uint32_t* reflOut; uint32_t* diffOut;
  const uint32_t* diffPrev; const unsigned long long* visDepth; uint32_t tilesX, rowBegin, rowEnd, carryMask;
  const uint32_t* tileWords;
  RayRec* spawnRays; HitKey* spawnHits; uint32_t* spawnCount; const float* cosSin;
  float* accRefl; float* accDiff;
};

enum ShadePass { SHADE_FINAL = 0, SHADE_SPAWN = 1, SHADE_FINAL_DEEP = 2, SHADE_ACCUM = 3, SHADE_SPAWN_ACCUM = 4 };
constexpr bool shadeSpawns(int pass) { return pass == SHADE_SPAWN || pass == SHADE_SPAWN_ACCUM; }
constexpr bool shadeAccumulates(int pass) { return pass == SHADE_ACCUM || pass == SHADE_SPAWN_ACCUM; }

RT_DEV f3 reflectionDepth1(const EnvRef& env, f2 rghMtl, f3 N, f3 V, f3 color) {
  const float level = calcMipFromRoughness(rghMtl.x, (float)env.mips);
  const float a = rghMtl.x * rghMtl.x;
  const f3 R = reflect3(-V, N);
  const f3 dir = lerp3(N, R, (1.0f - a) * (sqrtf(1.0f - a) + a));
  const float NoL = dot3(N, dir);
  if (NoL <= 0.0f) return mk3(0.0f, 0.0f, 0.0f);
  const f3 e = environment(env, dir, level);
  const f3 f0 = mk3(lerpf(0.04f, color.x, rghMtl.y), lerpf(0.04f, color.y, rghMtl.y), lerpf(0.04f, color.z, rghMtl.y));
  const float NoV = saturatef(dot3(N, V));
  return e * envBRDFApprox(f0, rghMtl.x, NoV);
}

RT_DEV uint32_t quadTileWord(const uint32_t* words, uint32_t tile32, uint32_t tilesX, uint32_t tilesY) {
  const uint32_t superX = (tilesX + 1u) >> 1, tx = (tile32 % superX) * 2u, ty = (tile32 / superX) * 2u;
  const uint32_t i0 = ty * tilesX + tx;
  const bool right = tx + 1u < tilesX, down = ty + 1u < tilesY;
  const uint32_t i1 = right ? i0 + 1u : i0, i2 = down ? i0 + tilesX : i0, i3 = right && down ? i0 + tilesX + 1u : i0;
  uint32_t a, b, c, d;
  asm volatile("s_load_dword %0, %4, %5\n\ts_load_dword %1, %4, %6\n\ts_load_dword %2, %4, %7\n\ts_load_dword %3, %4, %8\n\ts_waitcnt lgkmcnt(0)"
               : "=&s"(a), "=&s"(b), "=&s"(c), "=&s"(d)
               : "s"(words), "s"(RT_SGPR(i0 * 4u)), "s"(RT_SGPR(i1 * 4u)), "s"(RT_SGPR(i2 * 4u)), "s"(RT_SGPR(i3 * 4u)) : "memory");
  return a | b | c | d;
}
template <int RATE, int PASS, bool WIDE = false>
__global__ void __launch_bounds__(256, RT_GEN_MIN_BLOCKS) shadeKernel(const FrameParams* __restrict__ fpp, ShadeArgs A) {
  const FrameParams& fp = *fpp;
  const EnvRef env{A.env, A.envSize, A.envMips, A.envMipOffset};
  const uint32_t tile = blockIdx.x;
  { uint32_t word;
    if constexpr (RATE == 1) asm volatile("s_load_dword %0, %1, %2\n\ts_waitcnt lgkmcnt(0)" : "=s"(word) : "s"(A.tileWords), "s"(tile * 4u) : "memory");
    else word = quadTileWord(A.tileWords, tile, A.tilesX, (A.rowEnd - A.rowBegin + 15u) / 16u);
    if (word == 0u) return; }
  const uint32_t bin = tile * 4u + (threadIdx.x >> 6);
  if (RATE == 1 && A.carryMask != 0u) {
    const uint32_t lane = threadIdx.x & 63u, wave = threadIdx.x >> 6;
    const uint32_t px = (tile % A.tilesX) * 16u + (wave & 1u) * 8u + (lane & 7u);
    const uint32_t py = A.rowBegin + (tile / A.tilesX) * 16u + (wave >> 1) * 8u + (lane >> 3);
    if (px < fp.W && py < A.rowEnd) {
      const size_t pix = (size_t)py * fp.W + px;
      const uint32_t vis = (uint32_t)A.visDepth[pix];
      if (vis != 0u && ((A.carryMask >> ((vis - 1u) >> 24)) & 1u)) A.diffOut[pix] = A.diffPrev[pix];
    }
  }
  const uint32_t count = min(A.binCount[bin] & 0xFFu, A.binSlots);
  uint32_t spawned = 0u;
  for (uint32_t i = threadIdx.x & 63u; i < count; i += 64u) {
    const size_t slot = (size_t)bin * A.binSlots + i;
    const float4* rp = reinterpret_cast<const float4*>(A.rays + slot);
    const float4 q0 = rp[0], q1 = rp[1], q2 = rp[2];
    const float4 ra = make_float4(q0.x, q0.y, q0.z, RT_RAY_TMIN), rb = make_float4(q0.w, q1.x, q1.y, RT_RAY_TMAX), rw = make_float4(q2.x, q2.y, q2.z, 0.0f);
    const uint4 rc = make_uint4(__float_as_uint(q1.z), __float_as_uint(q1.w), __float_as_uint(q2.w), 0u);
    const uint32_t hitId = hitKeyId(A.hits[slot]);
    const f3 dir = mk3(rb.x, rb.y, rb.z);
    const bool diffuseGroup = (rc.z & 1u) != 0u;
    const uint32_t srcInst = rc.y >> 24;
    f3 col;
    bool child = false; RayRec cr;
    if (hitId == 0xFFFFFFFFu) col = environmentLevel0(env, dir);
    else {
      const float m = fp.mat.RoughMetals[srcInst][1];
      const f3 preset = mk3(fp.mat.BaseColors[srcInst][0] * m, fp.mat.BaseColors[srcInst][1] * m, fp.mat.BaseColors[srcInst][2] * m);
      if (!diffuseGroup && preset.x <= 0.0f && preset.y <= 0.0f && preset.z <= 0.0f) col = preset;
      else {
        const uint32_t hInst = hitId >> 24;
        uint32_t hPrim = hitId & 0xFFFFFFu;
        asm volatile("" : "+v"(hPrim));
        const Tri3 v = getVertices(hInst ? A.fat1 : A.fat0, hPrim);
        float ht, hb1 = 0.0f, hb2 = 0.0f;
        woopTestVerts(toObject(ra.x, ra.y, ra.z, rb.x, rb.y, rb.z, hInst ? fp.invWorld[1] : fp.invWorld[0]), v.pos[0], v.pos[1], v.pos[2], ht, hb1, hb2);
        const Attrib a = interpAttrib(v, hb1, hb2);
        const f3 N = normalize3(mulDir(a.Nrm, cbLoad3x3(hInst ? fp.g.WorldIT1 : fp.g.WorldITs0)));
        const f2 rm = getRoughMetal(fp.mat, hInst, a.UV);
        f3 color = mk3(fp.mat.BaseColors[hInst][0], fp.mat.BaseColors[hInst][1], fp.mat.BaseColors[hInst][2]);
        const f3 V = -dir;
        if constexpr (!shadeSpawns(PASS)) {
          if (rm.y > 0.5f) col = reflectionDepth1(env, rm, N, V, color);
          else {
            if (diffuseGroup) color = color * (1.0f - rm.y);
            const f3 irr = evaluateSHIrradiance(A.sh, N);
            col = mk3(irr.x / RT_PI, irr.y / RT_PI, irr.z / RT_PI) * color;
          }
        } else {
          const f3 P = mk3(ra.x + ht * rb.x, ra.y + ht * rb.y, ra.z + ht * rb.z);
          float xiY, cosPhi, sinPhi;
          if constexpr (WIDE) sampleParamWide(fp, A.cosSin, rc.x, xiY, cosPhi, sinPhi);
          else {
            uint32_t s = rng(rc.x); s += fp.g.FrameIndex; s = rng(s); s %= 256u;
            xiY = (float)(rng(s) & 0xffffu) / 65536.0f; cosPhi = A.cosSin[s]; sinPhi = A.cosSin[256 + s];
          }
          const uint32_t toDiffImage = (rc.z ^ (rc.z >> 1)) & 1u;
          f3 w, L;
          if (rm.y > 0.5f) {
            const bool vndf = (fp.flags & RT_FLAG_VNDF) != 0u;
            const f3 Hh = reflectionHalfVector(vndf, N, V, rm.x * rm.x, cosPhi, sinPhi, xiY);
            L = reflect3(-V, Hh);
            const float NoL = dot3(N, L);
            if (NoL <= 0.0f) col = mk3(0.0f, 0.0f, 0.0f);
            else { w = reflectionWeight(vndf, N, V, Hh, NoL, rm, color); child = true; cr.flags = toDiffImage << 1; }
          } else {
            if (diffuseGroup) color = color * (1.0f - rm.y);
            L = diffuseDirection(N, cosPhi, sinPhi, xiY);
            w = color; child = true; cr.flags = 1u | ((toDiffImage ^ 1u) << 1);
          }
          if (child) {
            cr.ox = P.x; cr.oy = P.y; cr.oz = P.z; cr.dx = L.x; cr.dy = L.y; cr.dz = L.z;
            cr.pixel = rc.x; cr.skip = hitId;
            cr.wx = rw.x * w.x; cr.wy = rw.y * w.y; cr.wz = rw.z * w.z;
          }
        }
      }
    }
// ... 236 lines not shown
  RT_HIP(hipStreamSynchronize(nullptr));
  return 0;
}

int launchRayTrace(rtggx_context* c, const FrameParams& fp, hipStream_t sGen, hipStream_t s, hipEvent_t done) {
  uint32_t rb, re;
  passRows(fp, ROWS_GBUFFER, rb, re);
  if (re <= rb) return 0;
  const uint32_t tilesX = (fp.W + 15) / 16, tilesY = (re - rb + 15) / 16;
  const bool quad = c->rayRate == 4u;
  const uint32_t quadX = (tilesX + 1u) / 2u, quadY = (tilesY + 1u) / 2u;
  if ((fp.mat.RoughMetals[0][1] < 1.0f || fp.mat.RoughMetals[1][1] < 1.0f) && c->binSlots < RT_BIN) {
    setError("rtggx_ray_trace: a material with metallic below 1 (a diffuse ray per pixel as well) but ray bins of %u slots: rtggx_update_frame sizes them", c->binSlots); return -1;
  }
  GenArgs G;
  const InputSet& set = c->cur();
  { const uint32_t thenFrame = c->frameCounter + 2u;
    VisTarget& vn = c->visOf(thenFrame);
    G.visNext = vn.depth; G.zeroNext0 = c->largeCountBase + (thenFrame & 1u); G.zeroNext1 = c->next().splitCount;
    vn.cleared.frame = thenFrame; vn.cleared.rows[0] = rb; vn.cleared.rows[1] = re;
    if (c->traceShare > 0.93f) c->traversalBound = true; else if (c->traceShare < 0.89f) c->traversalBound = false;
    G.visDirty = c->tileWords(rb, re); c->traceTileWords = quad ? c->visDirtyOnes : G.visDirty;
    G.visDirtyNextOut = vn.dirty;
    G.visDirtyNext = c->useTileWords && !c->traversalBound && vn.flags.rows[0] == rb && vn.flags.rows[1] == re ? vn.dirty : c->visDirtyOnes;
    vn.flags.rows[0] = rb; vn.flags.rows[1] = re;
  }
  G.visDepth = c->curVis().depth; G.depthOut = set.depth32; G.normalOut = set.normal; G.roughMetalOut = set.roughMetal; G.velocityOut = set.velocity; G.reflOut = set.rtRefl; G.diffOut = set.rtDiff;
  G.roughMetalPrev = c->prev().roughMetal;
  G.diffPrev = c->genCarriesDiff ? c->prev().rtDiff : nullptr;
  G.fat0 = c->mesh[0].fat; G.fat1 = c->mesh[1].fat;
  G.env = c->env.texels; G.envMipOffset = c->dEnvMipOffset; G.envSize = c->env.size; G.envMips = c->env.mips; G.cosSin = c->sampleTable();
  G.rays = (RayRec*)set.rayQueue.get(); G.hits = (HitKey*)set.hitQueue.get(); G.binCount = set.binCount; G.binSlots = c->binSlots; G.frameRays = c->rayCounter32;
  G.tilesX = tilesX; G.numTiles = tilesX * tilesY; G.rowBegin = rb; G.rowEnd = re;
  const uint32_t splitWork = c->splitWork, splitMaxShift = c->splitMaxShift;
  const uint32_t numBins = quad ? quadX * quadY * 4u : G.numTiles * 4u;
  const uint32_t sliceShift = chooseSliceShift(c, true, numBins);
  c->lastTraceSmall = c->forcePlacement >= 0 ? c->forcePlacement == 1 : (sliceShift > 0u || c->lastFrameRays < RT_WIDE_RAYS);
  const bool adaptive = splitWork != 0u && sliceShift == 0u;
  const uint32_t splitCap = !adaptive ? 0u : c->splitCapForced != 0xFFFFFFFFu ? c->splitCapForced
                          : c->splitDemand == 0u ? 0u : ((c->splitDemand + c->splitDemand / 8u + 64u + 31u) / 32u) * 32u;
  G.binWork = adaptive ? c->binWork : nullptr; G.splitList = set.splitList; G.splitCount = set.splitCount;
  G.frontWork = RT_SPLIT_FRONT < splitWork ? RT_SPLIT_FRONT : splitWork;
  G.splitWork = splitWork; G.splitMaxShift = splitMaxShift < 3u ? splitMaxShift : 3u; G.splitCap = splitCap < RT_SPLIT_CAP ? splitCap : RT_SPLIT_CAP;
  { SkyChain::GenFacts now;
    now.frame = c->frameCounter; now.rows[0] = rb; now.rows[1] = re; now.rate = c->rayRate; now.sliceShift = sliceShift; now.tilesX = tilesX; now.tilesY = tilesY;
    now.adaptive = adaptive; now.stream = sGen;
    memcpy(now.camera, fp.rg.ProjToWorld, 64); memcpy(now.camera + 16, fp.rg.EyePt, 16);
    G.skyEpoch = c->sky.rayGeneration(now); }
  if (c->sky.takeWrapped()) { const int r = clearSkyWordsAfterWrap(c); if (r) return r; }
  G.skyPrev = c->prev().skyRun; G.skyOut = set.skyRun; G.skyPrevRun = c->sky.prevRunThreshold(RT_SKY_PREV_RUN, RT_SKY_RUN_CAP);
  FrameEvents& ev = c->frameEvents(c->frameCounter);
  const FrameParams* genParams = c->dParams + c->slot;
  if (c->samples > 1u) {
    FrameParams* const sp = c->sppParams + (size_t)c->slot * RTGGX_MAX_SAMPLES_PER_PIXEL;
    hipLaunchKernelGGL(sampleParamsKernel, dim3(1), dim3(256), 0, sGen, genParams, sp, c->samples);
    genParams = sp;
  }
  const bool wide = c->sampleSet > RTGGX_MIN_SAMPLE_SET;
  launch(wide ? (quad ? rayGenKernel<4, true> : rayGenKernel<1, true>) : quad ? rayGenKernel<4> : rayGenKernel<1>, dim3(quad ? numBins : G.numTiles), dim3(256), sGen, nullptr, sGen != s ? ev.gen : nullptr, genParams, G);
  ev.genFrame = 0u; ev.genStream = sGen;
  if (sGen != s) {
    RT_HIP(hipStreamWaitEvent(s, ev.gen, 0));
    ev.genFrame = c->frameCounter;
  }
  if (c->timing) hipEventRecord(c->tev[11], s);
  const bool ring = c->kernelRing && c->kevCount < c->kevBegin.size() && (c->ringTick++ % c->ringStride) == 0u;
  const TraceQueue q{G.rays, G.hits, G.binCount, G.binSlots, nullptr};
  c->traceGrid[0] = numBins; c->traceGrid[1] = quad ? quadX : tilesX; c->traceGrid[2] = quad ? quadY : tilesY; c->traceGrid[3] = sliceShift;
  { const int r = launchTrace(c, fp, s, q, numBins, true, quad ? quadX : tilesX, quad ? quadY : tilesY, sliceShift, adaptive ? (int)G.splitCap : -1,
                              ring ? c->kevBegin[c->kevCount] : nullptr, ring ? c->kevEnd[c->kevCount] : done); if (r) return r; }
  if (c->timing) hipEventRecord(c->tev[12], s);
  if (ring) ++c->kevCount;
  if (done && ring) hipEventRecord(done, s);
  RT_HIP(hipGetLastError());
  return 0;
}

static void (*const kShade[3][2])(const FrameParams*, ShadeArgs) = {
    {shadeKernel<1, SHADE_FINAL>, shadeKernel<4, SHADE_FINAL>}, {shadeKernel<1, SHADE_SPAWN>, shadeKernel<4, SHADE_SPAWN>},
    {shadeKernel<1, SHADE_FINAL_DEEP>, shadeKernel<4, SHADE_FINAL_DEEP>}};
static void (*const kShadeSpawnWide[2])(const FrameParams*, ShadeArgs) = {shadeKernel<1, SHADE_SPAWN, true>, shadeKernel<4, SHADE_SPAWN, true>};
static int launchShadeSamples(rtggx_context* c, const FrameParams& fp, hipStream_t s, hipEvent_t done, ShadeArgs S, uint32_t numTiles, int spillPart) {
  const uint32_t N = c->samples, depth = c->maxDepth;
  const bool wide = c->sampleSet > RTGGX_MIN_SAMPLE_SET;
  if (!c->sppAcc || !c->sppParams) { setError("rtggx_ray_trace: %u samples per pixel without their buffers", N); return -1; }
  if (c->sppStream && c->sppStream != s) { RT_HIP(hipEventRecord(c->evSpp, c->sppStream)); RT_HIP(hipStreamWaitEvent(s, c->evSpp, 0)); }
  c->sppStream = s;
  const InputSet& set = c->cur();
  const FrameParams* const sp = c->sppParams + (size_t)c->slot * RTGGX_MAX_SAMPLES_PER_PIXEL;
  S.accRefl = c->sppAcc; S.accDiff = c->sppAcc + 3u * (size_t)c->W * c->H;
  SampleGenArgs G;
  G.visDepth = S.visDepth; G.fat0 = S.fat0; G.fat1 = S.fat1; G.cosSin = S.cosSin;
  G.rays = S.spawnRays; G.hits = S.spawnHits; G.binCount = S.spawnCount; G.binSlots = S.binSlots;
  G.tileWords = S.tileWords; G.tilesX = S.tilesX; G.rowBegin = S.rowBegin; G.rowEnd = S.rowEnd;
  const uint32_t* const map = c->sampleMapWords();
  if (map && (S.rowBegin != 0u || S.rowEnd != c->H)) { setError("rtggx_ray_trace: a sample map on rows [%u,%u) of %u", S.rowBegin, S.rowEnd, c->H); return -1; }
  SampleGenArgsMapped GM;
  static_cast<SampleGenArgs&>(GM) = G; GM.sampleMap = map; GM.sample = 0u;
  const TraceQueue q{S.rays, S.spawnHits, S.binCount, S.binSlots, nullptr};
  const bool sunHits = c->sun.on && c->sunReflections, lightHits = c->lights.count > 0u && c->lightReflections;
  if (sunHits || lightHits) { const int r = beginSunHits(c, s, false, sunHits, lightHits); if (r) return r; }
  for (uint32_t k = 0; k < N; ++k) {
    for (uint32_t level = 0; level < depth; ++level) {
      if (k > 0 && level == 0) {
        if (map) { GM.sample = k; launch(wide ? sampleGenKernel<true, true> : sampleGenKernel<false, true>, dim3(numTiles), dim3(256), s, nullptr, nullptr, sp + k, GM); }
        else launch(wide ? sampleGenKernel<true> : sampleGenKernel<false>, dim3(numTiles), dim3(256), s, nullptr, nullptr, sp + k, G);
      }
      if (k > 0 || level > 0) {
        const int r = launchTrace(c, fp, s, q, c->traceGrid[0], true, c->traceGrid[1], c->traceGrid[2], c->traceGrid[3], -1, nullptr, nullptr, spillPart);
        if (r) return r;
      }
      const HitPass hp{s, q, S.fat0, S.fat1, S.tileWords, numTiles, spillPart, true, S.accRefl, S.accDiff, fp.g.FrameIndex * N + k, level};
      if (sunHits) { const int r = launchSunHits(c, fp, hp); if (r) return r; }
      if (lightHits) { const int r = launchLightHits(c, fp, hp); if (r) return r; }
      launch(level + 1u < depth ? (wide ? shadeKernel<1, SHADE_SPAWN_ACCUM, true> : shadeKernel<1, SHADE_SPAWN_ACCUM>) : shadeKernel<1, SHADE_ACCUM>, dim3(numTiles), dim3(256), s, nullptr, nullptr, sp + k, S);
      S.carryMask = 0u;
      RT_HIP(hipGetLastError());
    }
  }
  ResolveArgs R;
  R.visDepth = S.visDepth; R.accRefl = S.accRefl; R.accDiff = S.accDiff; R.reflOut = set.rtRefl; R.diffOut = set.rtDiff;
  R.tileWords = S.tileWords; R.tilesX = S.tilesX; R.rowBegin = S.rowBegin; R.rowEnd = S.rowEnd;
  R.diffMask = (fp.mat.RoughMetals[0][1] < 1.0f ? 1u : 0u) | (fp.mat.RoughMetals[1][1] < 1.0f ? 2u : 0u);
  R.scale = 1.0f / (float)N;
  if (map) {
    ResolveArgsMapped RM;
    static_cast<ResolveArgs&>(RM) = R; RM.sampleMap = reinterpret_cast<const uint8_t*>(map); RM.samples = N;
    launch(resolveSamplesKernel<true>, dim3(numTiles), dim3(256), s, nullptr, done, c->dParams + c->slot, RM);
  } else launch(resolveSamplesKernel<false>, dim3(numTiles), dim3(256), s, nullptr, done, c->dParams + c->slot, R);
  RT_HIP(hipGetLastError());
  return 0;
}
int launchShade(rtggx_context* c, const FrameParams& fp, hipStream_t s, hipEvent_t done) {
  uint32_t rb, re;
  passRows(fp, ROWS_GBUFFER, rb, re);
  if (re <= rb) return 0;
  const uint32_t tilesX = (fp.W + 15) / 16, numTiles = tilesX * ((re - rb + 15) / 16);
  const InputSet& set = c->cur();
  ShadeArgs S;
  S.diffPrev = c->prev().rtDiff; S.visDepth = c->curVis().depth; S.tilesX = tilesX; S.rowBegin = rb; S.rowEnd = re;
  S.carryMask = (fp.mat.RoughMetals[0][1] >= 1.0f ? 1u : 0u) | (fp.mat.RoughMetals[1][1] >= 1.0f ? 2u : 0u);
  if (c->genCarriesDiff) S.carryMask = 0u;
  S.tileWords = c->tileWords(rb, re);
  const bool quad = c->rayRate == 4u;
  const uint32_t grid = quad ? ((tilesX + 1u) / 2u) * ((re - rb + 31u) / 32u) : numTiles;
  if (quad) S.carryMask = 0u;
  S.rays = (const RayRec*)set.rayQueue.get(); S.hits = (const HitKey*)set.hitQueue.get(); S.binCount = set.binCount; S.binSlots = c->binSlots;
  S.fat0 = c->mesh[0].fat; S.fat1 = c->mesh[1].fat;
  S.env = c->env.texels; S.envMipOffset = c->dEnvMipOffset; S.envSize = c->env.size; S.envMips = c->env.mips; S.sh = c->sh;
  S.reflOut = set.rtRefl; S.diffOut = set.rtDiff;
  S.spawnRays = (RayRec*)set.rayQueue.get(); S.spawnHits = (HitKey*)set.hitQueue.get(); S.spawnCount = set.binCount; S.cosSin = c->sampleTable();
  S.accRefl = nullptr; S.accDiff = nullptr;
  const FrameParams* const dfp = c->dParams + c->slot;
  const uint32_t depth = c->maxDepth;
  const int spillPart = s == c->streamMain ? 2 : (int)c->traceSpillHalf;
  if (c->samples > 1u && !quad) return launchShadeSamples(c, fp, s, done, S, numTiles, spillPart);
  const bool sunHits = c->sun.on && c->sunReflections && !quad, lightHits = c->lights.count > 0u && c->lightReflections && !quad, anyHits = sunHits || lightHits;
  float* sums[2] = {nullptr, nullptr};
  if (anyHits) {
    const int r = beginSunHits(c, s, true, sunHits, lightHits); if (r) return r;
    sums[0] = c->sunHitSums; sums[1] = c->sunHitSums + 4u * (size_t)c->W * c->H;
  }
  for (uint32_t level = 0; level < depth; ++level) {
    const TraceQueue q{S.rays, S.spawnHits, S.binCount, S.binSlots, nullptr};
    if (level > 0) {
      const int r = launchTrace(c, fp, s, q, c->traceGrid[0], true, c->traceGrid[1], c->traceGrid[2], c->traceGrid[3], -1, nullptr, nullptr, spillPart);
      if (r) return r;
      S.carryMask = 0u;
    }
    const HitPass hp{s, q, S.fat0, S.fat1, S.tileWords, numTiles, spillPart, false, sums[0], sums[1], fp.g.FrameIndex, level};
    if (sunHits) { const int r = launchSunHits(c, fp, hp); if (r) return r; }
    if (lightHits) { const int r = launchLightHits(c, fp, hp); if (r) return r; }
    const int pass = level + 1u < depth ? SHADE_SPAWN : level == 0 ? SHADE_FINAL : SHADE_FINAL_DEEP;
    launch(pass == SHADE_SPAWN && c->sampleSet > RTGGX_MIN_SAMPLE_SET ? kShadeSpawnWide[quad] : kShade[pass][quad], dim3(grid), dim3(256), s, nullptr, pass == SHADE_SPAWN || anyHits ? nullptr : done, dfp, S);
    RT_HIP(hipGetLastError());
  }
  if (anyHits) return launchSunHitResolve(c, s, c->sunHitSums, S.tileWords, tilesX, rb, re, done);
  return 0;
}

int launchReconstruct(rtggx_context* c, const FrameParams& fp, hipStream_t s) {
  uint32_t rb, re;
  passRows(fp, ROWS_GBUFFER, rb, re);
  if (re <= rb) return 0;
  const uint32_t tilesX = (fp.W + 15) / 16, numTiles = tilesX * ((re - rb + 15) / 16);
  const InputSet& set = c->cur();
  ReconArgs R;
  R.visDepth = c->curVis().depth; R.normal = set.normal; R.roughMetal = set.roughMetal; R.depth32 = set.depth32;
  R.reflOut = set.rtRefl; R.diffOut = set.rtDiff;
  R.diffPrev = c->prev().rtDiff;
  const uint32_t metal = (fp.mat.RoughMetals[0][1] >= 1.0f ? 1u : 0u) | (fp.mat.RoughMetals[1][1] >= 1.0f ? 2u : 0u);
  R.carryMask = c->genCarriesDiff ? 0u : metal; R.diffMask = ~metal & 3u;
  R.tileWords = c->tileWords(rb, re); R.tilesX = tilesX; R.rowBegin = rb; R.rowEnd = re;
  hipLaunchKernelGGL(reconstructKernel, dim3(numTiles), dim3(256), 0, s, c->dParams + c->slot, R);
  RT_HIP(hipGetLastError());
  return 0;
}

__global__ void fillTestQueue(const float* __restrict__ rays, uint32_t n, uint32_t binSlots, RayRec* q0, HitKey* keys, uint32_t* binCount, float2* tRange) {
  const uint32_t i = blockIdx.x * blockDim.x + threadIdx.x;
  if (i % binSlots == 0 && i < n) binCount[i / binSlots] = n - i < binSlots ? n - i : binSlots;
  if (i >= n) return;
  const float* r = rays + 8 * (size_t)i;
  RayRec rr;
  rr.ox = r[0]; rr.oy = r[1]; rr.oz = r[2]; rr.dx = r[3]; rr.dy = r[4]; rr.dz = r[5];
  rr.pixel = 0u; rr.skip = 0xFFFFFFFFu; rr.flags = 0u; rr.wx = rr.wy = rr.wz = 0.0f;
  q0[i] = rr;
  tRange[i] = make_float2(r[6], r[7]);
  keys[i] = hitKey(r[7], 0xFFFFFFFFu);
}
__global__ void exportTestHits(const FrameParams* __restrict__ fpp, const RayRec* __restrict__ rays, const HitKey* __restrict__ hits, uint32_t n,
                               const float4* __restrict__ fat0, const float4* __restrict__ fat1, float* __restrict__ out) {
  const uint32_t i = blockIdx.x * blockDim.x + threadIdx.x;
  if (i >= n) return;
  const HitKey k = hits[i];
  const uint32_t id = hitKeyId(k);
  float* o = out + 6 * (size_t)i;
  const bool valid = id != 0xFFFFFFFFu;
  float t = hitKeyT(k), b1 = 0.0f, b2 = 0.0f;
  if (valid) {
    const RayRec rr = rays[i];
    const uint32_t inst = id >> 24;
    uint32_t prim = id & 0xFFFFFFu;
    asm volatile("" : "+v"(prim));
    const Tri3 v = getVertices(inst ? fat1 : fat0, prim);
    woopTestVerts(toObject(rr.ox, rr.oy, rr.oz, rr.dx, rr.dy, rr.dz, inst ? fpp->invWorld[1] : fpp->invWorld[0]), v.pos[0], v.pos[1], v.pos[2], t, b1, b2);
  }
  o[0] = t; o[1] = u2f(valid ? id >> 24 : 0u); o[2] = u2f(valid ? id & 0xFFFFFFu : 0u); o[3] = b1; o[4] = b2; o[5] = valid ? 1.0f : 0.0f;
}
int launchTraceRays(rtggx_context* c, const FrameParams& fp, const float* dRays, uint32_t n, float* dOut, hipStream_t s) {
  if (!n) return 0;
  if (n > c->numBinsMax * c->binSlots) { setError("rtggx_trace_rays: at most %u rays per launch", c->numBinsMax * c->binSlots); return -1; }
  const uint32_t numBins = (((n + c->binSlots - 1u) / c->binSlots) + 3u) & ~3u;
  const InputSet& set = c->cur();
  RT_HIP(hipMemsetAsync(set.binCount, 0, (size_t)numBins * 4, s));
  if (!c->testRayRange) RT_HIP(alloc(c->testRayRange, (size_t)c->numBinsMax * RT_BIN * sizeof(float2)));
  hipLaunchKernelGGL(fillTestQueue, dim3((n + 255) / 256), dim3(256), 0, s, dRays, n, c->binSlots, (RayRec*)set.rayQueue.get(), (HitKey*)set.hitQueue.get(), set.binCount, (float2*)c->testRayRange.get());
  const TraceQueue q{(const RayRec*)set.rayQueue.get(), (HitKey*)set.hitQueue.get(), set.binCount, c->binSlots, (const float2*)c->testRayRange.get()};
  { const int r = launchTrace(c, fp, s, q, numBins, false, 0u, 0u, chooseSliceShift(c, false, numBins), -1); if (r) return r; }
  hipLaunchKernelGGL(exportTestHits, dim3((n + 255) / 256), dim3(256), 0, s, c->dParams + c->slot, (const RayRec*)set.rayQueue.get(), (const HitKey*)set.hitQueue.get(), n,
                     (const float4*)c->mesh[0].fat, (const float4*)c->mesh[1].fat, dOut);
  RT_HIP(hipGetLastError());
  return 0;
}

__global__ void exportOcclusion(const HitKey* __restrict__ hits, uint32_t n, uint32_t* __restrict__ out) {
  const uint32_t i = blockIdx.x * blockDim.x + threadIdx.x;
  if (i >= n) return;
  out[i] = hitKeyId(hits[i]) != 0xFFFFFFFFu ? 1u : 0u;
}
int launchTraceOcclusion(rtggx_context* c, const FrameParams& fp, const float* dRays, uint32_t n, uint32_t* dOut, hipStream_t s) {
  if (!n) return 0;
  if (n > c->numBinsMax * c->binSlots) { setError("rtggx_trace_occlusion: at most %u rays per launch", c->numBinsMax * c->binSlots); return -1; }
  const uint32_t numBins = (((n + c->binSlots - 1u) / c->binSlots) + 3u) & ~3u;
  const InputSet& set = c->cur();
  RT_HIP(hipMemsetAsync(set.binCount, 0, (size_t)numBins * 4, s));
  if (!c->testRayRange) RT_HIP(alloc(c->testRayRange, (size_t)c->numBinsMax * RT_BIN * sizeof(float2)));
// ... 108 lines not shown
```

raytracedggx_amd/csrc/rtggx_context.h:

```cpp
#pragma once
#include <hip/hip_runtime.h>
#include <hip/hip_ext.h>
#include <stdint.h>
#include <stdlib.h>
#include <string>
#include <utility>
#include <vector>
#include <memory>
#include "rtggx_device.h"
#include "rt_owned_hip.h"
#include "rt_sky_chain.h"

#ifndef RT_SETS
#define RT_SETS 4
#endif
#define RT_SLOTS (RT_SETS + 1)
#define RT_VIS_RING (RT_SETS + 2)
#define RT_VIS_CLEAR 0x00FFFFFF00000000ull
#define RT_SKY_PREV_RUN (RT_SETS + 2)
#define RT_SKY_V_RUN 2u
#define RT_SKY_WINDOW_RUN 1u
#define RT_SETTLED 1u
#define RT_SETTLED_SKIPPED 2u
#define RT_SETTLED_BORDER 0xFFFFFFFFu
#define RT_SKY_RUN_CAP 255u
namespace rt {

struct TraceQueue;
struct ShadowQueue {
  DevBuf<void> rays, hits, range; DevBuf<uint32_t> count; uint32_t slots = 0;
  int ensure(uint32_t numBins, uint32_t binSlots, bool withRange, bool& filled);
  void release();
  TraceQueue view() const;
};

#define RT_TREELET_LEVELS 3
struct BuildResult {
  uint32_t numRounds;
  uint32_t treelets[RT_TREELET_LEVELS];
  uint32_t topCount;
  uint32_t depth;
  uint32_t stack4, depth4, nodes4;
  uint32_t error;
  uint32_t itemCursor, roundCursor;
  uint32_t finalEntry, finalLds;
  float cost, pad2;
};
struct BvhTopo {
  DevBuf<uint32_t> order;
  DevBuf<int32_t> left, right, nodeParent, leafParent;
  DevBuf<float> nodeBox, triBox;
  DevBuf<uint32_t> cnt[RT_TREELET_LEVELS];
  DevBuf<uint32_t> roundBase;
  DevBuf<void> dTreelets, dRefitItems; DevBuf<uint32_t> dRefitRounds; DevBuf<int32_t> treeletRoots;
  DevBuf<int32_t> topList, topRank;
  DevBuf<float4> cost4;
  DevBuf<int4> ent4; DevBuf<uint32_t> lvl4;
  DevBuf<BuildResult> dResult; PinnedBuf<BuildResult> hResult;
  BuildResult result{};
  uint32_t numTris = 0; int32_t root = -1;
  bool refittable = false;
};

struct MeshDev {
  MeshDev(); ~MeshDev();
  float* verts = nullptr;
  DevBuf<float> vertsOwn[RT_SETS]; float* vertsBuf[RT_SETS] = {};
  float4* fat = nullptr; DevBuf<float4> fatOwn[RT_SETS]; float4* fatBuf[RT_SETS] = {};
  uint32_t vertsVersion[RT_SETS] = {}, version = 0, latestSet = 0;
  bool deforming = false;
  PinnedBuf<float> stage[RT_SLOTS];
  uint32_t stageNext = 0; int pendingStage = -1;
  DevBuf<float> deviceStage[RT_SLOTS];
  uint32_t deviceStageNext = 0; int pendingDeviceStage = -1; Event evProduced, evStaged;
  BvhTopo topo;
  std::unique_ptr<struct BuildJob> job;
  bool wantRebuild = false;
  uint32_t topoVersion = 0, topoVersionOfSet[RT_SETS] = {};
  DevBuf<float> dCost;
  PinnedBuf<float> hCost;
  Event evCost; bool costInFlight = false;
  float builtCost = 0.0f, lastCost = 0.0f;
  uint32_t refits = 0, rebuilds = 0;
  DevBuf<uint32_t> indices;
  uint32_t numVerts = 0, numIndices = 0, numTris = 0;
  BvhNode* nodes = nullptr;
  Bvh4Node* nodes4 = nullptr;
  BvhTri* tris = nullptr;
  DevBuf<BvhNode> nodesOwn[RT_SETS]; DevBuf<Bvh4Node> nodes4Own[RT_SETS]; DevBuf<BvhTri> trisOwn[RT_SETS];
  BvhNode* nodesBuf[RT_SETS] = {}; Bvh4Node* nodes4Buf[RT_SETS] = {}; BvhTri* trisBuf[RT_SETS] = {};
  uint32_t topCount = 0; uint32_t topCountBuf[RT_SETS] = {};
  Bvh4Node* top = nullptr; DevBuf<Bvh4Node> topOwn[RT_SETS]; Bvh4Node* topBuf[RT_SETS] = {};
  int32_t root = -1;
  uint32_t depth = 0;
  uint32_t stack4 = 0;
  float bmin[3] = {0, 0, 0}, bmax[3] = {0, 0, 0};
};

struct EnvDev {
  DevBuf<uint2> texels;
  uint32_t size = 0, mips = 0;
  uint32_t mipOffset[16] = {};
  uint64_t totalTexels = 0;
};

struct FrameParams {
  RtggxCBGlobal g;
  RtggxRayGenConstants rg;
  RtggxCBPerObject po[2];
  RtggxCBMaterial mat;
  float invWorld[2][16];
  uint32_t W, H;
  uint32_t rowBegin, rowEnd;
  uint32_t flags;
  uint32_t sampleMask;
  uint32_t pad[2];
};
#define RT_FLAG_VNDF 1u

struct InputSet {
  DevBuf<uint32_t> normal, velocity, rtRefl, rtDiff;
  DevBuf<uint16_t> roughMetal;
  DevBuf<uint32_t> depth32;
  DevBuf<void> rayQueue, hitQueue;
  DevBuf<uint32_t> binCount;
  DevBuf<uint32_t> splitList; uint32_t* splitCount = nullptr;
  DevBuf<uint32_t> skyRun;
  Event evRead;
  bool readRecorded = false;
};

struct VisTarget {
  DevBuf<unsigned long long> depth;
  DevBuf<uint32_t> dirty;
  struct { uint32_t frame = 0, rows[2] = {0, 0}; } cleared;
  struct { uint32_t rows[2] = {0, 0}; uint32_t rasterFrame = 0; } flags;
};

struct FrameEvents {
  Event gen;
  uint32_t genFrame = 0;
  hipStream_t genStream = nullptr;
  Event trace;
  bool traceRecorded = false;
};

}

#ifndef RT_COLLAPSE_AREA_WEIGHT
#define RT_COLLAPSE_AREA_WEIGHT 1.0f
#define RT_COLLAPSE_TRIS_WEIGHT 0.0f
#endif
#define RT_MAX_PEERS 16

struct rtggx_context {
  int device = 0;
  uint32_t W = 0, H = 0;
  uint32_t rowBegin = 0, rowEnd = 0;
  uint32_t historyApron = 18;
  rt::DevBuf<uint32_t> histReach;
  rt::Stream ownMain; hipStream_t streamMain = nullptr, streamAS = nullptr;
  rt::Stream streamRefit;
  bool refitIssued = false;
  uint32_t frameCounter = 0;
  rt::FrameEvents frames[4];
  rt::FrameEvents& frameEvents(uint32_t f) { return frames[f & 3u]; }
  rt::Stream ownAS, ownVis;
  bool asyncCompute = true;
  hipStream_t streamVis = nullptr;
  rt::Event evVis;
  hipStream_t evVisStream = nullptr;
  rt::Event evAS;
  rt::Event evRefit;
  rt::Event evRT;
  int setReadDeferred = -1;
  double fenceWaitUs = 0.0; uint32_t fenceWaits = 0;
  int fuseToneMap = -1; bool toneMapDone = false, denoiseIssued = false;
  rt::DevBuf<uint32_t> exchangeTokens;
  float collapseWeights[2] = {RT_COLLAPSE_AREA_WEIGHT, RT_COLLAPSE_TRIS_WEIGHT};
  uint32_t peerWorld = 0; rt::DevBuf<void> dPeerTable; std::vector<rt::IpcMapping> ipcMapped;
  uint32_t lastPlacement[2] = {0, 0};
  int forcePlacement = -1;
  bool fltRflIsFltDff = false;
  bool externalStream = false;

  bool vndf = false;
  struct Sun { bool on = false; float L[3] = {}, E[3] = {}, T[3] = {}, B[3] = {}; } sun, sunRequested;
  rt::ShadowQueue sunQueue;
  struct SunAngle { float degrees = 0.0f, k = 0.0f; } sunAngle, sunAngleRequested;
  bool sunReflections = false, sunReflectionsRequested = false;
  rt::ShadowQueue sunHitQueue; rt::DevBuf<float> sunHitSums;
  hipStream_t sunHitStream = nullptr; rt::Event evSunHit;
  struct Lights { uint32_t count = 0; RtggxLight l[RTGGX_MAX_LIGHTS] = {}; } lights, lightsRequested;
  rt::ShadowQueue lightQueue; rt::DevBuf<float> lightSums;
  bool lightReflections = false, lightReflectionsRequested = false;
  rt::ShadowQueue lightHitQueue;
  uint32_t lightSampling = 0, lightSamplingRequested = 0;
  rt::DevBuf<float> lightPickDiff;
  uint32_t rayRate = 1;
  uint32_t maxDepth = 1, depthRequested = 1;
  uint32_t samples = 1, samplesRequested = 1;
  rt::DevBuf<float> sppAcc; rt::DevBuf<rt::FrameParams> sppParams;
  hipStream_t sppStream = nullptr; rt::Event evSpp;
  bool accumulate = false, accumulateRequested = false;
  uint32_t accumFrames = 0;
  rt::DevBuf<uint32_t> sampleMapBuf[2];
  int sampleMap = -1, sampleMapRequested = -1;
  const uint32_t* sampleMapWords() const { return sampleMap < 0 ? nullptr : sampleMapBuf[sampleMap].get(); }
  rt::DevBuf<float4> accRefl, accDiff; rt::DevBuf<uint2> converged;
  bool scoring = false, scoringRequested = false;
  rt::DevBuf<uint2> reference;
  rt::DevBuf<double> scorePartial[2]; rt::DevBuf<uint32_t> scoreCounts; uint32_t scoreStride = 0;
  rt::DevBuf<RtggxScore> scoreRing;
  uint64_t scoreIndex = 0, scoreRead = 0;
  uint32_t traceGrid[4] = {};
  float rebuildRatio = 1.2f; uint32_t rebuildSteps = 16;
  rt::MeshDev mesh[2];
  rt::EnvDev env;
  rt::DevBuf<float> sh;
  rt::DevBuf<float> cosSinTab;
  uint32_t sampleSet = RTGGX_MIN_SAMPLE_SET, sampleSetRequested = RTGGX_MIN_SAMPLE_SET;
  rt::DevBuf<float> cosSinWide[8];
  static uint32_t sampleSetSlot(uint32_t m) { uint32_t k = 0; while ((512u << k) < m) ++k; return k; }
  const float* sampleTable() const { return sampleSet > RTGGX_MIN_SAMPLE_SET ? cosSinWide[sampleSetSlot(sampleSet)] : cosSinTab; }

  rt::InputSet sets[RT_SETS];
  uint32_t setIndex = 0;
  uint32_t setAhead(uint32_t k) const { return (setIndex + k) % RT_SETS; }
  rt::InputSet& cur() { return sets[setIndex]; }
  rt::InputSet& prev() { return sets[setAhead(RT_SETS - 1u)]; }
  rt::InputSet& next() { return sets[setAhead(1u)]; }
  rt::VisTarget vis[RT_VIS_RING];
  rt::VisTarget& visOf(uint32_t frame) { return vis[frame % RT_VIS_RING]; }
  rt::VisTarget& curVis() { return visOf(frameCounter); }
  void selectSet(uint32_t i) {
    setIndex = i;
    largeTris = largeTrisBuf[frameCounter & 1u]; largeCount = largeCountBase ? largeCountBase + (frameCounter & 1u) : nullptr;
    for (auto& m : mesh) { m.verts = m.vertsBuf[i]; m.fat = m.fatBuf[i]; m.nodes = m.nodesBuf[i]; m.nodes4 = m.nodes4Buf[i]; m.top = m.topBuf[i]; m.topCount = m.topCountBuf[i]; m.tris = m.trisBuf[i]; }
    binWork = binWorkBuf[frameCounter & 1u]; rayCounter32 = rayCounterBuf + (frameCounter & 3u) * 256u;
  }
  rt::DevBuf<uint32_t> backbuffer;
  rt::DevBuf<uint2> tss[2], fltRfl, fltDff;
  uint32_t frameParity = 0;

  void* largeTris = nullptr; rt::DevBuf<void> largeTrisBuf[2];
  uint32_t* largeCount = nullptr;
  rt::DevBuf<uint32_t> largeCountBase;
  uint32_t* binWork = nullptr;
  rt::DevBuf<uint32_t> binWorkBuf[2];
  const uint32_t* tileWords(uint32_t rb, uint32_t re) {
    const rt::VisTarget& v = curVis();
    return useTileWords && !traversalBound && v.flags.rasterFrame == frameCounter && v.flags.rows[0] == rb && v.flags.rows[1] == re ? v.dirty.get() : visDirtyOnes.get();
  }
  rt::SkyChain sky;
  size_t skyTiles = 0;
  rt::DevBuf<uint32_t> settled[2]; uint32_t settledX = 0, settledY = 0, settledPitch = 0;
  size_t settledWords() const { return (size_t)(settledX + 2u) * settledPitch + 8u; }
  bool useTileWords = true;
  bool traversalBound = false;
  const uint32_t* traceTileWords = nullptr;
  rt::DevBuf<uint32_t> visDirtyOnes;
  uint32_t splitDemand = 0;
  uint32_t splitCapForced = 0xFFFFFFFFu;
  uint32_t splitWork = 0, splitMaxShift = 0;
  uint32_t largeCapacity = 0;

  uint32_t numBinsMax = 0, binSlots = 64;
  rt::DevBuf<void> testRayRange;
  rt::DevBuf<int32_t> stackOverflow;
  uint32_t spillEntries = 0;
  rt::DevBuf<void> dummyRecord;
  rt::DevBuf<uint32_t> dEnvMipOffset;
  bool lastTraceSmall = false; uint32_t traceSpillHalf = 0;
  hipStream_t shadeStream = nullptr;
  bool genCarriesDiff = false, shadeWroteDiff = false, lastFrameDiffuse = false;
  hipStream_t diffStream = nullptr;
  uint32_t numCUs = 256;
  uint32_t traceWaves = 12, traceWavesForced = 0; float traceShare = 0.0f; rt::DevBuf<unsigned long long> traceStamps; uint32_t traceStampLaunch = 0;
  unsigned long long traceStampSum = 0, traceStampStart = 0; uint32_t traceStampAt = 0, traceSampleLaunch = 0;
  uint32_t traceTrial = 0, traceCooldown = 0, traceWavesSince = 0; float traceTrialBase = 0.0f;

  rt::PinnedBuf<uint32_t> hostRayCounters;
  rt::Event evRayCounters; bool rayCountersInFlight = false; uint32_t traceLaunches = 0;
  uint32_t lastFrameRays = 0xFFFFFFFFu;
  uint32_t* rayCounter32 = nullptr;
  rt::DevBuf<uint32_t> rayCounterBuf;
  uint32_t* lastRayCounter32 = nullptr;
  rt::DevBuf<unsigned long long> rayCounter;

  rt::FrameParams slots[RT_SLOTS];
  uint32_t slot = 0;
  rt::DevBuf<rt::FrameParams> dParams;
  bool slotUploaded = false;
  bool slotRendered = false;
  RtggxCBMaterial material;
  float invWorld[2][16];
  bool haveConstants = false, asBuilt = false, shDone = false;

  bool timing = false;
  bool kernelRing = false;
  uint32_t ringStride = 1, ringTick = 0;
  std::vector<rt::Event> kevBegin, kevEnd;
  uint32_t kevCount = 0;
  rt::Event tev[16];
  bool timingsPending = false;
};

namespace rt {
enum RowPass { ROWS_GBUFFER , ROWS_VFILTER , ROWS_TEMPORAL , ROWS_FINAL };
inline void passRows(const FrameParams& fp, RowPass pass, uint32_t& b, uint32_t& e) {
  const uint32_t apron = pass == ROWS_GBUFFER ? 18u : pass == ROWS_VFILTER ? 2u : pass == ROWS_TEMPORAL ? 1u : 0u;
  b = fp.rowBegin > apron ? fp.rowBegin - apron : 0u;
  e = fp.rowEnd + apron < fp.H ? fp.rowEnd + apron : fp.H;
  if (fp.rowEnd <= fp.rowBegin) { b = e = 0; }
}
void setError(const char* fmt, ...);
#define RT_HIP(expr) do { hipError_t _e = (expr); if (_e != hipSuccess) { rt::setError("%s failed: %s (%s:%d)", #expr, hipGetErrorString(_e), __FILE__, __LINE__); return -2; } } while (0)
template <class... P, class... A>
inline void launch(void (*k)(P...), dim3 grid, dim3 block, hipStream_t s, hipEvent_t start, hipEvent_t stop, A&&... a) {
  if (start || stop) hipExtLaunchKernelGGL(k, grid, block, 0, s, start, stop, 0, static_cast<P>(a)...);
  else hipLaunchKernelGGL(k, grid, block, 0, s, static_cast<P>(a)...);
}

int uploadParams(rtggx_context* c, uint32_t slot, hipStream_t s);
int launchVisibility(rtggx_context* c, const FrameParams& fp, hipStream_t s, hipEvent_t done = nullptr);
int buildLbvh(rtggx_context* c, uint32_t slot, hipStream_t s);
int startRebuild(rtggx_context* c, uint32_t slot, uint32_t set);
int continueRebuild(rtggx_context* c, uint32_t slot, hipStream_t s, uint32_t maxSteps, bool* swapped);
int prepareRebuild(rtggx_context* c, uint32_t slot);
void abandonRebuild(rtggx_context* c, uint32_t slot);
int refitLbvh(rtggx_context* c, uint32_t slot, uint32_t set, hipStream_t s);
void freeBuildProducts(MeshDev& m);
int buildFatTris(rtggx_context* c, uint32_t slot, uint32_t set, hipStream_t s);
int launchRayTrace(rtggx_context* c, const FrameParams& fp, hipStream_t sGen, hipStream_t sTrace, hipEvent_t done = nullptr);
int launchShade(rtggx_context* c, const FrameParams& fp, hipStream_t s, hipEvent_t done = nullptr);
// ... 38 lines not shown
```

raytracedggx_amd/csrc/visibility.hip:

```cpp
#include "rtggx_context.h"
#include "rt_raster.h"

namespace rt {


struct RVert { long long X, Y; float z; bool ok; };

RT_DEV f4 clipVertex(const float* __restrict__ pos, const M4& wvp, float bx, float by) {
  f4 p = mulPoint(mk3(pos[0], pos[1], pos[2]), wvp);
  p.x += bx * p.w;
  p.y += by * p.w;
  return p;
}
RT_DEV RVert rasterVertex(f4 p, uint32_t W, uint32_t H) {
  RVert r; r.X = 0; r.Y = 0; r.z = 0.0f; r.ok = false;
  if (!(p.w > 0.0f)) return r;
  const float nx = p.x / p.w, ny = p.y / p.w;
  r.z = p.z / p.w;
  const float sx = (nx + 1.0f) * ((float)W * 0.5f);
  const float sy = (1.0f - ny) * ((float)H * 0.5f);
  const float fx = floorf(sx * 256.0f + 0.5f), fy = floorf(sy * 256.0f + 0.5f);
  if (!(fabsf(fx) < 1073741824.0f) || !(fabsf(fy) < 1073741824.0f)) return r;
  r.X = (long long)fx; r.Y = (long long)fy; r.ok = true;
  return r;
// ... 164 lines not shown
  for (uint32_t w = lane; w < total; w += 64u) {
    uint32_t lo = 0;
#pragma unroll
    for (uint32_t step = TPW / 2u; step > 0u; step >>= 1) if (prefix[lo + step] <= w) lo += step;
    const TriSetup& S = setup[lo];
    const uint32_t q = w - prefix[lo], bw = S.bwTl & 0xFFFFu;
    const uint32_t ry = (q * S.magic) >> 20, rx = q - ry * bw;
    const int32_t px = S.px0 + (int32_t)rx, py = S.py0 + (int32_t)ry;
    const int32_t X[3] = {S.X[0], S.X[1], S.X[2]}, Y[3] = {S.Y[0], S.Y[1], S.Y[2]};
    const double z0 = (double)S.z[0], dz1 = (double)S.z[1] - z0, dz2 = (double)S.z[2] - z0;
    const unsigned long long key = fragmentKey(px * 256 + 128, py * 256 + 128, X, Y, (S.bwTl >> 16) & 1u, (S.bwTl >> 17) & 1u, (S.bwTl >> 18) & 1u,
                                               S.invA, z0, dz1, dz2, S.word);
    if (key == ~0ull) continue;
    unsigned long long* dst = vd + (size_t)py * fp.W + (size_t)px;
#if RT_RASTER_PREREAD
    const unsigned long long before = *dst;
    if (key < before) { atomicMin(dst, key); if (before == RT_VIS_CLEAR) dirty[(((uint32_t)py - rowBegin) >> 4) * tilesX + ((uint32_t)px >> 4)] = 1u; }
#else
    atomicMin(dst, key);
    dirty[(((uint32_t)py - rowBegin) >> 4) * tilesX + ((uint32_t)px >> 4)] = 1u;
#endif
  }
}

#ifndef RT_LARGE_ROWS
#define RT_LARGE_ROWS 16
#endif
__global__ void __launch_bounds__(256) rasterLarge(uint32_t W, uint32_t rowBegin, uint32_t rowEnd, unsigned long long* __restrict__ vd, const LargeTri* __restrict__ large,
                                                   const uint32_t* __restrict__ largeCount, uint32_t largeCap, uint32_t* __restrict__ dirty, uint32_t tilesX) {
  const uint32_t px = blockIdx.x * 64 + (threadIdx.x & 63);
  const uint32_t y0 = rowBegin + blockIdx.y * RT_LARGE_ROWS, py0 = y0 + (threadIdx.x >> 6);
  const uint32_t n = min(*largeCount, largeCap);
  const int32_t bx0 = (int32_t)(blockIdx.x * 64) * 256 + 128, bx1 = bx0 + 63 * 256, by0 = (int32_t)y0 * 256 + 128, by1 = by0 + (RT_LARGE_ROWS - 1) * 256;
  const int32_t PX = (int32_t)px * 256 + 128;
  unsigned long long best[RT_LARGE_ROWS / 4];
#pragma unroll
  for (int k = 0; k < RT_LARGE_ROWS / 4; ++k) best[k] = ~0ull;
  for (uint32_t i = 0; i < n; ++i) {
    const LargeTri lt = large[i];
    const int32_t minX = min(lt.X[0], min(lt.X[1], lt.X[2])), maxX = max(lt.X[0], max(lt.X[1], lt.X[2]));
    const int32_t minY = min(lt.Y[0], min(lt.Y[1], lt.Y[2])), maxY = max(lt.Y[0], max(lt.Y[1], lt.Y[2]));
    if (maxX < bx0 || minX > bx1 || maxY < by0 || minY > by1) continue;
    const double z0 = (double)lt.z[0], dz1 = (double)lt.z[1] - z0, dz2 = (double)lt.z[2] - z0;
#pragma unroll
    for (int k = 0; k < RT_LARGE_ROWS / 4; ++k) {
      const unsigned long long key = fragmentKey(PX, (int32_t)(py0 + 4u * k) * 256 + 128, lt.X, lt.Y, lt.tl & 1u, (lt.tl >> 1) & 1u, (lt.tl >> 2) & 1u, lt.invA, z0, dz1, dz2, lt.word);
      best[k] = key < best[k] ? key : best[k];
    }
  }
  if (px >= W) return;
#pragma unroll
  for (int k = 0; k < RT_LARGE_ROWS / 4; ++k) {
    const uint32_t py = py0 + 4u * k;
    if (py < rowEnd && best[k] != ~0ull) {
      unsigned long long* dst = vd + (size_t)py * W + px;
      if (best[k] < *dst) { *dst = best[k]; dirty[((py - rowBegin) >> 4) * tilesX + (px >> 4)] = 1u; }
    }
  }
}

__global__ void unpackVisDepthKernel(const unsigned long long* __restrict__ vd, uint32_t* __restrict__ vis, uint32_t* __restrict__ depth, uint32_t n) {
  const uint32_t i = blockIdx.x * blockDim.x + threadIdx.x;
  if (i < n) { const unsigned long long k = vd[i]; vis[i] = (uint32_t)k; depth[i] = (uint32_t)(k >> 32); }
}
__global__ void packVisDepthKernel(unsigned long long* __restrict__ vd, const uint32_t* __restrict__ vis, const uint32_t* __restrict__ depth, uint32_t n) {
  const uint32_t i = blockIdx.x * blockDim.x + threadIdx.x;
  if (i < n) vd[i] = ((unsigned long long)depth[i] << 32) | vis[i];
}

int launchVisibility(rtggx_context* c, const FrameParams& fp, hipStream_t s, hipEvent_t done) {
  uint32_t rb, re;
  passRows(fp, ROWS_GBUFFER, rb, re);
  const uint32_t begin = rb * fp.W, end = re * fp.W;
  if (end <= begin) return 0;
  VisTarget& v = c->curVis();
  uint32_t* const dirty = v.dirty;
  const uint32_t tilesX = (fp.W + 15) / 16, tilesY = (re - rb + 15) / 16;
  if (!(v.cleared.frame == c->frameCounter && v.cleared.rows[0] <= rb && v.cleared.rows[1] >= re)) {
    hipLaunchKernelGGL(clearVisDepth, dim3((end - begin + 1023) / 1024), dim3(256), 0, s, v.depth, begin, end, c->largeCount, c->cur().splitCount);
    RT_HIP(hipMemsetAsync(dirty, 0, (size_t)tilesX * tilesY * 4, s));
  }
  v.flags.rows[0] = rb; v.flags.rows[1] = re; v.flags.rasterFrame = c->frameCounter;
  v.cleared.frame = 0u;
  const uint32_t nt = c->mesh[0].numTris + c->mesh[1].numTris;
  FrameParams* const dst = c->slotUploaded ? (FrameParams*)nullptr : c->dParams + c->slot;
  c->slotUploaded = true;
  const dim3 grid(nt ? (nt + 4u * RT_RASTER_TPW - 1u) / (4u * RT_RASTER_TPW) : 1u);
  hipLaunchKernelGGL(rasterSmall, grid, dim3(256), 0, s, fp, dst, rb, re, (const float*)c->mesh[0].verts, (const uint32_t*)c->mesh[0].indices, c->mesh[0].numTris,
                     (const float*)c->mesh[1].verts, (const uint32_t*)c->mesh[1].indices, c->mesh[1].numTris, v.depth, (LargeTri*)c->largeTris, c->largeCount, c->largeCapacity, dirty, tilesX);
  if (nt) {
    const dim3 lgrid((fp.W + 63) / 64, (re - rb + RT_LARGE_ROWS - 1) / RT_LARGE_ROWS);
    launch(rasterLarge, lgrid, dim3(256), s, nullptr, done, fp.W, rb, re, v.depth, c->largeTris, c->largeCount, c->largeCapacity, dirty, tilesX);
  } else if (done) hipEventRecord(done, s);
  RT_HIP(hipGetLastError());
  return 0;
}

int unpackVisDepth(rtggx_context* c, uint32_t* dVis, uint32_t* dDepth, hipStream_t s) {
  const uint32_t n = c->W * c->H;
  hipLaunchKernelGGL(unpackVisDepthKernel, dim3((n + 255) / 256), dim3(256), 0, s, c->curVis().depth, dVis, dDepth, n);
  RT_HIP(hipGetLastError());
  return 0;
}
int packVisDepth(rtggx_context* c, const uint32_t* dVis, const uint32_t* dDepth, hipStream_t s) {
  const uint32_t n = c->W * c->H;
  RT_HIP(hipMemsetAsync(c->curVis().dirty, 0xFF, (size_t)((c->W + 15) / 16) * ((c->H + 15) / 16 + 1) * 4, s));
  hipLaunchKernelGGL(packVisDepthKernel, dim3((n + 255) / 256), dim3(256), 0, s, c->curVis().depth, dVis, dDepth, n);
  RT_HIP(hipGetLastError());
  return 0;
}

}
```

Baseline: 3306 Mrays/s.

## Bound shade and horizontal filter launches to projected mesh screen footprint

Each frame the host projects every mesh's world bounding box to screen, builds a convex hull and derives per-tile-row spans plus a bounding rectangle. The shade kernel (rate 1) and the horizontal spatial filter kernels then launch only over that rectangle and exit early for blocks outside the row span, so sky-only tiles no longer need a block launched. It adds host-side hull math per frame and extra span checks in the kernels. It falls back to full grids for deforming meshes, multi-sample or quad rate, or multiple uses of one visibility pass. With the ground plane present the footprint may cover most of the screen.

```diff
diff --git a/include/rtggx.h b/include/rtggx.h
--- a/include/rtggx.h
+++ b/include/rtggx.h
@@ -167,6 +167,9 @@
 int  rtggx_debug_fuse_tone_map(rtggx_context* ctx, int mode);
 int  rtggx_debug_placement(rtggx_context* ctx, int force_small, uint32_t* key, uint32_t* where);
 int  rtggx_debug_tile_words(rtggx_context* ctx, int enable);
+int  rtggx_debug_launch_bound(rtggx_context* ctx, int enable);
+#define RTGGX_LAUNCH_BOUND_INFO 20
+int  rtggx_debug_launch_bound_read(rtggx_context* ctx, uint32_t* spans, uint32_t* tile_words, uint32_t capacity, uint32_t* info);
 int  rtggx_debug_static_sky(rtggx_context* ctx, int enable);
 int  rtggx_debug_sky_runs(rtggx_context* ctx, uint32_t* runs, uint32_t capacity, uint32_t* tiles_x, uint32_t* tiles_y, uint32_t* threshold);
 int  rtggx_debug_settled_sky(rtggx_context* ctx, int enable);
diff --git a/raytracedggx_amd/capi.py b/raytracedggx_amd/capi.py
--- a/raytracedggx_amd/capi.py
+++ b/raytracedggx_amd/capi.py
@@ -31,7 +31,7 @@
            "rtggx_transform_sh", "rtggx_render_visibility", "rtggx_ray_trace", "rtggx_denoise", "rtggx_tone_map", "rtggx_sync",
            "rtggx_ray_count", "rtggx_get_timings", "rtggx_enable_timing", "rtggx_buffer_size", "rtggx_readback", "rtggx_buffer_ptr",
            "rtggx_upload", "rtggx_frame_parity", "rtggx_bvh_root", "rtggx_trace_rays", "rtggx_ray_total", "rtggx_kernel_times", "rtggx_debug_counters", "rtggx_debug_trace_split", "rtggx_debug_trace_residency", "rtggx_get_stream", "rtggx_set_history_peers", "rtggx_history_ipc_export", "rtggx_history_ipc_open",
-           "rtggx_set_async_compute", "rtggx_set_history_apron", "rtggx_history_overreach", "rtggx_copy_bandwidth", "rtggx_refit_as", "rtggx_refit_as_device", "rtggx_refit_stats", "rtggx_set_refit_policy", "rtggx_set_sampler", "rtggx_set_ray_rate", "rtggx_set_max_recursion_depth", "rtggx_set_samples_per_pixel", "rtggx_debug_fuse_tone_map", "rtggx_debug_placement", "rtggx_debug_tile_words", "rtggx_debug_static_sky", "rtggx_debug_settled_sky", "rtggx_debug_settled_words", "rtggx_debug_sky_runs", "rtggx_debug_collapse_weights", "rtggx_debug_fence_wait", "rtggx_debug_shader_clock", "rtggx_debug_environment",
+           "rtggx_set_async_compute", "rtggx_set_history_apron", "rtggx_history_overreach", "rtggx_copy_bandwidth", "rtggx_refit_as", "rtggx_refit_as_device", "rtggx_refit_stats", "rtggx_set_refit_policy", "rtggx_set_sampler", "rtggx_set_ray_rate", "rtggx_set_max_recursion_depth", "rtggx_set_samples_per_pixel", "rtggx_debug_fuse_tone_map", "rtggx_debug_placement", "rtggx_debug_tile_words", "rtggx_debug_launch_bound", "rtggx_debug_launch_bound_read", "rtggx_debug_static_sky", "rtggx_debug_settled_sky", "rtggx_debug_settled_words", "rtggx_debug_sky_runs", "rtggx_debug_collapse_weights", "rtggx_debug_fence_wait", "rtggx_debug_shader_clock", "rtggx_debug_environment",
            "rtggx_set_accumulation", "rtggx_reset_accumulation", "rtggx_accumulated_frames", "rtggx_present_accumulation", "rtggx_set_sample_set",
            "rtggx_set_reference", "rtggx_reference_from_accumulation", "rtggx_set_scoring", "rtggx_read_scores",
            "rtggx_set_env_image", "rtggx_generate_env_mips", "rtggx_prefilter_env",
@@ -239,6 +239,23 @@
     def tile_words(self, enable):
         self._check(self.L.rtggx_debug_tile_words(self.h, 1 if enable else 0))
 
+    def launch_bound(self, enable):
+        self.L.rtggx_debug_launch_bound.argtypes = [C.c_void_p, C.c_int]
+        self._check(self.L.rtggx_debug_launch_bound(self.h, 1 if enable else 0))
+
+    def launch_bound_read(self):
+        cap = ((self.W + 15) // 16) * ((self.H + 15) // 16 + 1)
+        spans, words, info = np.zeros(cap, np.uint32), np.zeros(cap, np.uint32), np.zeros(20, np.uint32)
+        self.L.rtggx_debug_launch_bound_read.argtypes = [C.c_void_p, C.c_void_p, C.c_void_p, C.c_uint32, C.c_void_p]
+        self._check(self.L.rtggx_debug_launch_bound_read(self.h, _p(spans), _p(words), cap, _p(info)))
+        i = [int(x) for x in info]
+        tx, ty = i[1], i[2]
+        rows = min(ty, 136)
+        return {"full": bool(i[0]), "tiles_x": tx, "tiles_y": ty, "row0": i[3], "rows": i[4], "rect_x0": i[5], "rect_w": i[6],
+                "shade_grid": (i[7], i[8]), "shade_full": (i[9], i[10]), "filter_grid": (i[11], i[12]), "filter_full": (i[13], i[14]),
+                "in_force": bool(i[15]), "words_valid": bool(i[16]), "pass_rows": (i[17], i[18]), "tiles": i[19],
+                "spans": np.stack([spans[:rows] & 0xFFFF, spans[:rows] >> 16], axis=1).astype(np.int64), "words": words[:tx * ty].reshape(ty, tx)}
+
     def static_sky(self, enable):
         self._check(self.L.rtggx_debug_static_sky(self.h, 1 if enable else 0))
 
diff --git a/raytracedggx_amd/csrc/debug.hip b/raytracedggx_amd/csrc/debug.hip
--- a/raytracedggx_amd/csrc/debug.hip
+++ b/raytracedggx_amd/csrc/debug.hip
@@ -48,6 +48,28 @@
   RT_CHECK_CTX(c);
   c->useTileWords = enable != 0;
   c->sky.breakRuns(SkyBreak::TileWordsSwitch);
+  return 0;
+}
+int rtggx_debug_launch_bound(rtggx_context* c, int enable) {
+  RT_CHECK_CTX(c);
+  c->useLaunchBound = enable != 0;
+  return 0;
+}
+int rtggx_debug_launch_bound_read(rtggx_context* c, uint32_t* spans, uint32_t* tileWords, uint32_t capacity, uint32_t* info) {
+  RT_CHECK_CTX(c);
+  if (!info) { setError("rtggx_debug_launch_bound_read: null info"); return -1; }
+  const VisTarget& v = c->curVis();
+  const LaunchBound& b = v.bound;
+  const uint32_t rowsInTable = b.tilesY < RT_BOUND_ROWS ? b.tilesY : RT_BOUND_ROWS, n = b.tilesX * b.tilesY;
+  if ((spans && capacity < rowsInTable) || (tileWords && (capacity < n || n > c->skyTiles))) { setError("rtggx_debug_launch_bound_read: room for %u spans, %u words", rowsInTable, n); return -1; }
+  RT_HIP(syncStreams(c));
+  if (spans) for (uint32_t r = 0; r < rowsInTable; ++r) spans[r] = (uint32_t)b.spans.row[r].x0 | ((uint32_t)b.spans.row[r].w << 16);
+  if (tileWords && n) RT_HIP(hipMemcpy(tileWords, v.dirty, (size_t)n * 4, hipMemcpyDeviceToHost));
+  const rtggx_context::LastBound& L = c->lastBound;
+  const uint32_t out[RTGGX_LAUNCH_BOUND_INFO] = {b.full ? 1u : 0u, b.tilesX, b.tilesY, b.row0, b.rows, b.rectX0, b.rectW,
+    L.shadeGrid[0], L.shadeGrid[1], L.shadeFull[0], L.shadeFull[1], L.filterGrid[0], L.filterGrid[1], L.filterFull[0], L.filterFull[1],
+    L.frame == c->frameCounter && !L.bound.full ? 1u : 0u, v.flags.rasterFrame == c->frameCounter ? 1u : 0u, v.flags.rows[0], v.flags.rows[1], b.tiles()};
+  memcpy(info, out, sizeof out);
   return 0;
 }
 int rtggx_debug_static_sky(rtggx_context* c, int enable) {
diff --git a/raytracedggx_amd/csrc/denoise.hip b/raytracedggx_amd/csrc/denoise.hip
--- a/raytracedggx_amd/csrc/denoise.hip
+++ b/raytracedggx_amd/csrc/denoise.hip
@@ -141,12 +141,20 @@
   return TM3(unpackR11G11B10F(MODE >= 2 ? T.rtDiff[ti] : T.rtRefl[ti]));
 }
 
+struct FilterBound { uint32_t bx0, by0; LaunchSpans spans; };
+RT_DEV bool outsideBound(const FilterBound& B, uint32_t bx, uint32_t gridY) {
+  const uint32_t span = reinterpret_cast<const uint32_t*>(B.spans.row)[min(gridY >> 2, RT_BOUND_ROWS - 1u)];
+  const uint32_t x0 = span & 0xFFFFu, w = span >> 16;
+  return bx * 4u >= x0 + w || bx * 4u + 3u < x0;
+}
 template <int MODE>
-__global__ void __launch_bounds__(256) spatialDirectKernel(Targets T) {
+__global__ void __launch_bounds__(256) spatialDirectKernel(Targets T, FilterBound B) {
   constexpr bool vertical = (MODE & 1) != 0;
   constexpr bool diffuse = MODE >= 2;
-  const int x = blockIdx.x * 64 + (threadIdx.x & 63);
-  const int y = T.rowBegin + blockIdx.y * 4 + (threadIdx.x >> 6);
+  const uint32_t bx = vertical ? blockIdx.x : B.bx0 + blockIdx.x, by = vertical ? blockIdx.y : B.by0 + blockIdx.y;
+  if (!vertical && outsideBound(B, bx, blockIdx.y)) return;
+  const int x = bx * 64 + (threadIdx.x & 63);
+  const int y = T.rowBegin + by * 4 + (threadIdx.x >> 6);
   if (x >= T.W || y >= T.rowEnd) return;
   const size_t pix = (size_t)y * T.W + x;
   const GTexel gc = loadG(T.normal, T.roughMetal, T.depth32, x, y, T.W, T.H);
@@ -168,9 +176,11 @@
 
 typedef float V4 __attribute__((ext_vector_type(4)));
 template <int MODE>
-__global__ void __launch_bounds__(256) spatialTiledKernel(Targets T) {
+__global__ void __launch_bounds__(256) spatialTiledKernel(Targets T, FilterBound B) {
   constexpr bool vertical = (MODE & 1) != 0;
   constexpr bool diffuse = MODE >= 2;
+  const uint32_t bx = vertical ? blockIdx.x : B.bx0 + blockIdx.x, by = vertical ? blockIdx.y : B.by0 + blockIdx.y;
+  if (!vertical && outsideBound(B, bx, blockIdx.y)) return;
   constexpr int BW = vertical ? RT_VBW : 64, BH = vertical ? RT_VBH : 4;
   constexpr int TW = vertical ? RT_VBW : 96, TH = vertical ? RT_VBH + 2 * RT_RADIUS : 4;
   constexpr int PER = vertical ? BW * BH / 256 : 1, ROWSTEP = 256 / BW;
@@ -178,7 +188,7 @@
   __shared__ V4 smA[N], smB[N];
   __shared__ uint32_t roughLo, roughHi, unflagged;
   if (threadIdx.x == 0) { roughLo = 0xFFFFFFFFu; roughHi = 0u; unflagged = 0u; }
-  const int bx0 = blockIdx.x * BW, by0 = T.rowBegin + blockIdx.y * BH;
+  const int bx0 = bx * BW, by0 = T.rowBegin + by * BH;
   const int lx = threadIdx.x % BW, ly = threadIdx.x / BW;
   const int x = bx0 + lx;
 
@@ -641,21 +651,36 @@
   { SkyChain::VFacts now;
     now.frame = c->frameCounter; now.gbufferRow0 = (uint32_t)TV.tileRow0; now.rows[0] = (uint32_t)TV.rowBegin; now.rows[1] = (uint32_t)TV.rowEnd; now.fltRflNull = TVr.fltRfl == nullptr;
     if (c->sky.reflectionV(now) && useLds) { TVr.skyRun = c->cur().skyRun; TVr.skyEpoch = c->sky.epoch(); } }
+  FilterBound FB;
+  const dim3 fullH = grid(TH, 64, 4);
+  dim3 gridH = fullH;
+  { const LaunchBound& bound = c->launchBound((uint32_t)TH.rowBegin, (uint32_t)TH.rowEnd);
+    const BoundGrid bg = filterGrid(bound, (uint32_t)TH.rowBegin, (uint32_t)TH.rowEnd);
+    FB.bx0 = bg.x0; FB.by0 = bg.y0; FB.spans = gridSpans(bound);
+    if (!bound.full) gridH = dim3(bg.nx, bg.ny);
+    if (c->lastBound.frame != c->frameCounter) { c->lastBound.shadeGrid[0] = c->lastBound.shadeGrid[1] = c->lastBound.shadeFull[0] = c->lastBound.shadeFull[1] = 0u; }
+    c->lastBound.bound = bound; c->lastBound.frame = c->frameCounter;
+    c->lastBound.filterGrid[0] = gridH.x; c->lastBound.filterGrid[1] = gridH.y; c->lastBound.filterFull[0] = fullH.x; c->lastBound.filterFull[1] = fullH.y; }
+  const bool anyH = gridH.x > 0u && gridH.y > 0u;
   if (useLds) {
-    hipLaunchKernelGGL(spatialTiledKernel<0>, grid(TH, 64, 4), block, 0, s, TH); mark(4);
-    hipLaunchKernelGGL(spatialTiledKernel<1>, grid(TV, RT_VBW, RT_VBH), block, 0, s, TVr); mark(5);
-    if (anyDiffuse) hipLaunchKernelGGL(spatialTiledKernel<2>, grid(TH, 64, 4), block, 0, s, TH);
+    if (anyH) hipLaunchKernelGGL(spatialTiledKernel<0>, gridH, block, 0, s, TH, FB);
+    mark(4);
+    hipLaunchKernelGGL(spatialTiledKernel<1>, grid(TV, RT_VBW, RT_VBH), block, 0, s, TVr, FB); mark(5);
+    if (anyDiffuse && anyH) hipLaunchKernelGGL(spatialTiledKernel<2>, gridH, block, 0, s, TH, FB);
     mark(6);
-    if (anyDiffuse) hipLaunchKernelGGL(spatialTiledKernel<3>, grid(TV, RT_VBW, RT_VBH), block, 0, s, TV);
+    if (anyDiffuse) hipLaunchKernelGGL(spatialTiledKernel<3>, grid(TV, RT_VBW, RT_VBH), block, 0, s, TV, FB);
     mark(7);
   } else if (!anyDiffuse) {
-    hipLaunchKernelGGL(spatialDirectKernel<0>, grid(TH, 64, 4), block, 0, s, TH); mark(4);
-    hipLaunchKernelGGL(spatialDirectKernel<1>, grid(TV, 64, 4), block, 0, s, TVr); mark(5); mark(6); mark(7);
+    if (anyH) hipLaunchKernelGGL(spatialDirectKernel<0>, gridH, block, 0, s, TH, FB);
+    mark(4);
+    hipLaunchKernelGGL(spatialDirectKernel<1>, grid(TV, 64, 4), block, 0, s, TVr, FB); mark(5); mark(6); mark(7);
   } else {
-    hipLaunchKernelGGL(spatialDirectKernel<0>, grid(TH, 64, 4), block, 0, s, TH); mark(4);
-    hipLaunchKernelGGL(spatialDirectKernel<1>, grid(TV, 64, 4), block, 0, s, TV); mark(5);
-    hipLaunchKernelGGL(spatialDirectKernel<2>, grid(TH, 64, 4), block, 0, s, TH); mark(6);
-    hipLaunchKernelGGL(spatialDirectKernel<3>, grid(TV, 64, 4), block, 0, s, TV); mark(7);
+    if (anyH) hipLaunchKernelGGL(spatialDirectKernel<0>, gridH, block, 0, s, TH, FB);
+    mark(4);
+    hipLaunchKernelGGL(spatialDirectKernel<1>, grid(TV, 64, 4), block, 0, s, TV, FB); mark(5);
+    if (anyH) hipLaunchKernelGGL(spatialDirectKernel<2>, gridH, block, 0, s, TH, FB);
+    mark(6);
+    hipLaunchKernelGGL(spatialDirectKernel<3>, grid(TV, 64, 4), block, 0, s, TV, FB); mark(7);
   }
   Targets TTs = TT;
   { SkyChain::TemporalFacts now;
diff --git a/raytracedggx_amd/csrc/frame.hip b/raytracedggx_amd/csrc/frame.hip
--- a/raytracedggx_amd/csrc/frame.hip
+++ b/raytracedggx_amd/csrc/frame.hip
@@ -179,6 +179,7 @@
   if (!c->haveConstants || !c->asBuilt) { setError("rtggx_ray_trace: %s", c->asBuilt ? "no frame constants" : "rtggx_build_as has not been called"); return -1; }
   if (!c->env.texels) { setError("rtggx_ray_trace: no environment map"); return -1; }
   { const int r = ensureParams(c); if (r) return r; }
+  ++c->visUses;
   const uint32_t f = c->frameCounter;
   const FrameParams& fp = c->slots[c->slot];
   const Placement P = placeFrame(c, fp, f);
diff --git a/raytracedggx_amd/csrc/raytrace.hip b/raytracedggx_amd/csrc/raytrace.hip
--- a/raytracedggx_amd/csrc/raytrace.hip
+++ b/raytracedggx_amd/csrc/raytrace.hip
@@ -390,6 +390,8 @@
   const uint32_t* tileWords;
   RayRec* spawnRays; HitKey* spawnHits; uint32_t* spawnCount; const float* cosSin;
   float* accRefl; float* accDiff;
+  uint32_t boundX0, boundRow0;
+  LaunchSpans spans;
 };
 
 enum ShadePass { SHADE_FINAL = 0, SHADE_SPAWN = 1, SHADE_FINAL_DEEP = 2, SHADE_ACCUM = 3, SHADE_SPAWN_ACCUM = 4 };
@@ -424,7 +426,13 @@
 __global__ void __launch_bounds__(256, RT_GEN_MIN_BLOCKS) shadeKernel(const FrameParams* __restrict__ fpp, ShadeArgs A) {
   const FrameParams& fp = *fpp;
   const EnvRef env{A.env, A.envSize, A.envMips, A.envMipOffset};
-  const uint32_t tile = blockIdx.x;
+  uint32_t tile = blockIdx.x;
+  if constexpr (RATE == 1) {
+    const uint32_t span = reinterpret_cast<const uint32_t*>(A.spans.row)[min(blockIdx.y, RT_BOUND_ROWS - 1u)];
+    const uint32_t tx = A.boundX0 + blockIdx.x, ty = A.boundRow0 + blockIdx.y;
+    if (tx - (span & 0xFFFFu) >= (span >> 16)) return;
+    tile = ty * A.tilesX + tx;
+  }
   { uint32_t word;
     if constexpr (RATE == 1) asm volatile("s_load_dword %0, %1, %2\n\ts_waitcnt lgkmcnt(0)" : "=s"(word) : "s"(A.tileWords), "s"(tile * 4u) : "memory");
     else word = quadTileWord(A.tileWords, tile, A.tilesX, (A.rowEnd - A.rowBegin + 15u) / 16u);
@@ -827,6 +835,7 @@
 static void (*const kShadeSpawnWide[2])(const FrameParams*, ShadeArgs) = {shadeKernel<1, SHADE_SPAWN, true>, shadeKernel<4, SHADE_SPAWN, true>};
 static int launchShadeSamples(rtggx_context* c, const FrameParams& fp, hipStream_t s, hipEvent_t done, ShadeArgs S, uint32_t numTiles, int spillPart) {
   const uint32_t N = c->samples, depth = c->maxDepth;
+  const dim3 fullGrid(S.tilesX, numTiles / S.tilesX);
   const bool wide = c->sampleSet > RTGGX_MIN_SAMPLE_SET;
   if (!c->sppAcc || !c->sppParams) { setError("rtggx_ray_trace: %u samples per pixel without their buffers", N); return -1; }
   if (c->sppStream && c->sppStream != s) { RT_HIP(hipEventRecord(c->evSpp, c->sppStream)); RT_HIP(hipStreamWaitEvent(s, c->evSpp, 0)); }
@@ -858,7 +867,7 @@
       const HitPass hp{s, q, S.fat0, S.fat1, S.tileWords, numTiles, spillPart, true, S.accRefl, S.accDiff, fp.g.FrameIndex * N + k, level};
       if (sunHits) { const int r = launchSunHits(c, fp, hp); if (r) return r; }
       if (lightHits) { const int r = launchLightHits(c, fp, hp); if (r) return r; }
-      launch(level + 1u < depth ? (wide ? shadeKernel<1, SHADE_SPAWN_ACCUM, true> : shadeKernel<1, SHADE_SPAWN_ACCUM>) : shadeKernel<1, SHADE_ACCUM>, dim3(numTiles), dim3(256), s, nullptr, nullptr, sp + k, S);
+      launch(level + 1u < depth ? (wide ? shadeKernel<1, SHADE_SPAWN_ACCUM, true> : shadeKernel<1, SHADE_SPAWN_ACCUM>) : shadeKernel<1, SHADE_ACCUM>, fullGrid, dim3(256), s, nullptr, nullptr, sp + k, S);
       S.carryMask = 0u;
       RT_HIP(hipGetLastError());
     }
@@ -888,7 +897,13 @@
   if (c->genCarriesDiff) S.carryMask = 0u;
   S.tileWords = c->tileWords(rb, re);
   const bool quad = c->rayRate == 4u;
-  const uint32_t grid = quad ? ((tilesX + 1u) / 2u) * ((re - rb + 31u) / 32u) : numTiles;
+  const LaunchBound& bound = c->launchBound(rb, re);
+  const BoundGrid bg = shadeGrid(bound);
+  S.boundX0 = bg.x0; S.boundRow0 = bg.y0; S.spans = gridSpans(bound);
+  const dim3 grid = quad ? dim3(((tilesX + 1u) / 2u) * ((re - rb + 31u) / 32u)) : dim3(bg.nx, bg.ny);
+  c->lastBound.bound = bound; c->lastBound.frame = c->frameCounter;
+  c->lastBound.shadeGrid[0] = quad ? grid.x : bg.nx; c->lastBound.shadeGrid[1] = quad ? 1u : bg.ny; c->lastBound.shadeFull[0] = quad ? grid.x : tilesX; c->lastBound.shadeFull[1] = quad ? 1u : numTiles / tilesX;
+  c->lastBound.filterGrid[0] = c->lastBound.filterGrid[1] = c->lastBound.filterFull[0] = c->lastBound.filterFull[1] = 0u;
   if (quad) S.carryMask = 0u;
   S.rays = (const RayRec*)set.rayQueue.get(); S.hits = (const HitKey*)set.hitQueue.get(); S.binCount = set.binCount; S.binSlots = c->binSlots;
   S.fat0 = c->mesh[0].fat; S.fat1 = c->mesh[1].fat;
@@ -906,6 +921,7 @@
     const int r = beginSunHits(c, s, true, sunHits, lightHits); if (r) return r;
     sums[0] = c->sunHitSums; sums[1] = c->sunHitSums + 4u * (size_t)c->W * c->H;
   }
+  const bool empty = grid.x == 0u || grid.y == 0u;
   for (uint32_t level = 0; level < depth; ++level) {
     const TraceQueue q{S.rays, S.spawnHits, S.binCount, S.binSlots, nullptr};
     if (level > 0) {
@@ -917,7 +933,8 @@
     if (sunHits) { const int r = launchSunHits(c, fp, hp); if (r) return r; }
     if (lightHits) { const int r = launchLightHits(c, fp, hp); if (r) return r; }
     const int pass = level + 1u < depth ? SHADE_SPAWN : level == 0 ? SHADE_FINAL : SHADE_FINAL_DEEP;
-    launch(pass == SHADE_SPAWN && c->sampleSet > RTGGX_MIN_SAMPLE_SET ? kShadeSpawnWide[quad] : kShade[pass][quad], dim3(grid), dim3(256), s, nullptr, pass == SHADE_SPAWN || anyHits ? nullptr : done, dfp, S);
+    if (empty) { if (pass != SHADE_SPAWN && !anyHits && done) RT_HIP(hipEventRecord(done, s)); continue; }
+    launch(pass == SHADE_SPAWN && c->sampleSet > RTGGX_MIN_SAMPLE_SET ? kShadeSpawnWide[quad] : kShade[pass][quad], grid, dim3(256), s, nullptr, pass == SHADE_SPAWN || anyHits ? nullptr : done, dfp, S);
     RT_HIP(hipGetLastError());
   }
   if (anyHits) return launchSunHitResolve(c, s, c->sunHitSums, S.tileWords, tilesX, rb, re, done);
diff --git a/raytracedggx_amd/csrc/rt_launch_bound.h b/raytracedggx_amd/csrc/rt_launch_bound.h
--- /dev/null
+++ b/raytracedggx_amd/csrc/rt_launch_bound.h
@@ -0,0 +1,140 @@
+#pragma once
+#include <cmath>
+#include <cstdint>
+
+namespace rt {
+
+#define RT_BOUND_ROWS 136u
+#define RT_BOUND_MIN_W 1e-6f
+
+struct TileSpan { uint16_t x0, w; };
+struct LaunchSpans { TileSpan row[RT_BOUND_ROWS]; };
+
+struct LaunchBound {
+  LaunchSpans spans;
+  uint32_t tilesX = 0, tilesY = 0;
+  uint32_t row0 = 0, rows = 0;
+  uint32_t rectX0 = 0, rectW = 0;
+  bool full = true;
+  uint32_t tiles() const { uint32_t n = 0; for (uint32_t r = row0; r < row0 + rows && r < RT_BOUND_ROWS; ++r) n += spans.row[r].w; return full ? tilesX * tilesY : n; }
+};
+
+struct BoundInstance {
+  const float* worldViewProj = nullptr; const float* projBias = nullptr;
+  float bmin[3] = {0, 0, 0}, bmax[3] = {0, 0, 0};
+  bool present = false;
+  bool known = false;
+};
+
+inline void launchBoundFull(LaunchBound& b, uint32_t W, uint32_t rowBegin, uint32_t rowEnd) {
+  b.tilesX = (W + 15u) / 16u; b.tilesY = rowEnd > rowBegin ? (rowEnd - rowBegin + 15u) / 16u : 0u;
+  b.full = true; b.row0 = 0u; b.rows = b.tilesY; b.rectX0 = 0u; b.rectW = b.tilesX;
+  for (auto& s : b.spans.row) { s.x0 = 0u; s.w = 0xFFFFu; }
+}
+
+namespace bound_detail {
+struct P2 { double x, y; };
+inline double cross(const P2& o, const P2& a, const P2& b) { return (a.x - o.x) * (b.y - o.y) - (a.y - o.y) * (b.x - o.x); }
+inline int hull8(P2* p, int n, P2* h) {
+  for (int i = 1; i < n; ++i) { const P2 v = p[i]; int j = i; while (j > 0 && (p[j - 1].x > v.x || (p[j - 1].x == v.x && p[j - 1].y > v.y))) { p[j] = p[j - 1]; --j; } p[j] = v; }
+  int k = 0;
+  for (int i = 0; i < n; ++i) { while (k >= 2 && cross(h[k - 2], h[k - 1], p[i]) <= 0.0) --k; h[k++] = p[i]; }
+  for (int i = n - 2, t = k + 1; i >= 0; --i) { while (k >= t && cross(h[k - 2], h[k - 1], p[i]) <= 0.0) --k; h[k++] = p[i]; }
+  return k > 1 ? k - 1 : k;
+}
+}
+
+inline void computeLaunchBound(LaunchBound& b, const BoundInstance* inst, int numInst, uint32_t W, uint32_t H, uint32_t rowBegin, uint32_t rowEnd) {
+  using namespace bound_detail;
+  launchBoundFull(b, W, rowBegin, rowEnd);
+  if (b.tilesY == 0u || b.tilesY > RT_BOUND_ROWS || b.tilesX > 0xFFFFu) return;
+  int lo[RT_BOUND_ROWS], hi[RT_BOUND_ROWS];
+  for (uint32_t r = 0; r < b.tilesY; ++r) { lo[r] = 0x7FFFFFFF; hi[r] = -1; }
+  for (int n = 0; n < numInst; ++n) {
+    const BoundInstance& I = inst[n];
+    if (!I.present) continue;
+    if (!I.known) return;
+    const float* f = I.worldViewProj;
+    double absMax[3];
+    for (int k = 0; k < 3; ++k) {
+      if (!(std::isfinite(I.bmin[k]) && std::isfinite(I.bmax[k]) && I.bmin[k] <= I.bmax[k])) return;
+      absMax[k] = std::fmax(std::fabs((double)I.bmin[k]), std::fabs((double)I.bmax[k]));
+    }
+    for (int k = 0; k < 16; ++k) if (!std::isfinite(f[k])) return;
+    double S[4];
+    for (int j = 0; j < 4; ++j) S[j] = absMax[0] * std::fabs((double)f[j * 4]) + absMax[1] * std::fabs((double)f[j * 4 + 1]) + absMax[2] * std::fabs((double)f[j * 4 + 2]) + std::fabs((double)f[j * 4 + 3]);
+    P2 pts[8]; double wMin = 1e300, nMax = 0.0;
+    for (int c = 0; c < 8; ++c) {
+      const double p[3] = {(c & 1) ? I.bmax[0] : I.bmin[0], (c & 2) ? I.bmax[1] : I.bmin[1], (c & 4) ? I.bmax[2] : I.bmin[2]};
+      double clip[4];
+      for (int j = 0; j < 4; ++j) clip[j] = p[0] * f[j * 4] + p[1] * f[j * 4 + 1] + p[2] * f[j * 4 + 2] + f[j * 4 + 3];
+      if (!(clip[3] > (double)RT_BOUND_MIN_W + S[3] * 0x1p-21) || !(clip[2] >= S[2] * 0x1p-21)) return;
+      wMin = std::fmin(wMin, clip[3]);
+      const double nx = clip[0] / clip[3] + (double)I.projBias[0], ny = clip[1] / clip[3] + (double)I.projBias[1];
+      nMax = std::fmax(nMax, std::fmax(std::fabs(nx), std::fabs(ny)));
+      pts[c].x = (nx + 1.0) * ((double)W * 0.5); pts[c].y = (1.0 - ny) * ((double)H * 0.5);
+    }
+    const double E = (double)W * 0.5 * 0x1p-21 * ((std::fmax(S[0], S[1]) + nMax * S[3]) / wMin + 4.0 * (nMax + 1.0));
+    if (!(E < 64.0)) return;
+    const double margin = 1.0 + 1.0 / 512.0 + E;
+    P2 h[18];
+    const int nh = hull8(pts, 8, h);
+    for (uint32_t r = 0; r < b.tilesY; ++r) {
+      const double ya = (double)(rowBegin + 16u * r) - margin, yb = (double)(rowBegin + 16u * r + 16u) + margin;
+      double xa = 1e300, xb = -1e300;
+      for (int e = 0; e < nh; ++e) {
+        P2 p = h[e], q = h[(e + 1) % nh];
+        if (p.y > q.y) { const P2 t = p; p = q; q = t; }
+        if (q.y < ya || p.y > yb) continue;
+        double x0 = p.x, x1 = q.x;
+        if (q.y > p.y) {
+          const double s = (q.x - p.x) / (q.y - p.y);
+          if (p.y < ya) x0 = p.x + (ya - p.y) * s;
+          if (q.y > yb) x1 = p.x + (yb - p.y) * s;
+        }
+        xa = std::fmin(xa, std::fmin(x0, x1)); xb = std::fmax(xb, std::fmax(x0, x1));
+      }
+      if (xa > xb) continue;
+      const double px0 = std::floor(xa - margin), px1 = std::floor(xb + margin);
+      if (px1 < 0.0 || px0 >= (double)W) continue;
+      int t0 = (int)(std::fmax(px0, 0.0) / 16.0), t1 = (int)(std::fmin(px1, (double)W - 1.0) / 16.0);
+#ifdef RT_BOUND_SHRINK
+      ++t0; --t1;
+      if (t0 > t1) continue;
+#endif
+      if (t0 < lo[r]) lo[r] = t0;
+      if (t1 > hi[r]) hi[r] = t1;
+    }
+  }
+  b.full = false; b.row0 = 0u; b.rows = 0u;
+  int rx0 = 0x7FFFFFFF, rx1 = -1;
+  uint32_t first = b.tilesY, last = 0u;
+  for (uint32_t r = 0; r < RT_BOUND_ROWS; ++r) {
+    TileSpan& s = b.spans.row[r];
+    if (r < b.tilesY && lo[r] <= hi[r]) {
+      s.x0 = (uint16_t)lo[r]; s.w = (uint16_t)(hi[r] - lo[r] + 1);
+      if (lo[r] < rx0) rx0 = lo[r];
+      if (hi[r] > rx1) rx1 = hi[r];
+      if (r < first) first = r;
+      last = r;
+    } else { s.x0 = 0u; s.w = 0u; }
+  }
+  if (first < b.tilesY) { b.row0 = first; b.rows = last - first + 1u; b.rectX0 = (uint32_t)rx0; b.rectW = (uint32_t)(rx1 - rx0 + 1); }
+  else { b.row0 = 0u; b.rows = 0u; b.rectX0 = 0u; b.rectW = 0u; }
+}
+
+struct BoundGrid { uint32_t x0, y0, nx, ny; };
+inline LaunchSpans gridSpans(const LaunchBound& b) {
+  LaunchSpans t;
+  for (uint32_t i = 0; i < RT_BOUND_ROWS; ++i) t.row[i] = b.row0 + i < RT_BOUND_ROWS ? b.spans.row[b.row0 + i] : TileSpan{0u, 0u};
+  return t;
+}
+inline BoundGrid shadeGrid(const LaunchBound& b) { return {b.rectX0, b.row0, b.rectW, b.rows}; }
+inline BoundGrid filterGrid(const LaunchBound& b, uint32_t rowBegin, uint32_t rowEnd) {
+  if (b.rectW == 0u || b.rows == 0u) return {0u, 0u, 0u, 0u};
+  const uint32_t bx0 = b.rectX0 / 4u, bx1 = (b.rectX0 + b.rectW - 1u) / 4u;
+  const uint32_t blockRows = (rowEnd - rowBegin + 3u) / 4u, by0 = b.row0 * 4u, by1 = (b.row0 + b.rows) * 4u < blockRows ? (b.row0 + b.rows) * 4u : blockRows;
+  return {bx0, by0, bx1 - bx0 + 1u, by1 - by0};
+}
+
+}
diff --git a/raytracedggx_amd/csrc/rtggx_context.h b/raytracedggx_amd/csrc/rtggx_context.h
--- a/raytracedggx_amd/csrc/rtggx_context.h
+++ b/raytracedggx_amd/csrc/rtggx_context.h
@@ -10,6 +10,7 @@
 #include "rtggx_device.h"
 #include "rt_owned_hip.h"
 #include "rt_sky_chain.h"
+#include "rt_launch_bound.h"
 
 #ifndef RT_SETS
 #define RT_SETS 4
@@ -135,6 +136,7 @@
   DevBuf<uint32_t> dirty;
   struct { uint32_t frame = 0, rows[2] = {0, 0}; } cleared;
   struct { uint32_t rows[2] = {0, 0}; uint32_t rasterFrame = 0; } flags;
+  LaunchBound bound;
 };
 
 struct FrameEvents {
@@ -251,6 +253,16 @@
   const uint32_t* tileWords(uint32_t rb, uint32_t re) {
     const rt::VisTarget& v = curVis();
     return useTileWords && !traversalBound && v.flags.rasterFrame == frameCounter && v.flags.rows[0] == rb && v.flags.rows[1] == re ? v.dirty.get() : visDirtyOnes.get();
+  }
+  bool useLaunchBound = true;
+  uint32_t visUses = 0;
+  rt::LaunchBound fullBound;
+  struct LastBound { rt::LaunchBound bound; uint32_t shadeGrid[2] = {0, 0}, shadeFull[2] = {0, 0}, filterGrid[2] = {0, 0}, filterFull[2] = {0, 0}; uint32_t frame = 0; } lastBound;
+  const rt::LaunchBound& launchBound(uint32_t rb, uint32_t re) {
+    const rt::VisTarget& v = curVis();
+    if (useLaunchBound && visUses <= 1u && rayRate == 1u && samples == 1u && tileWords(rb, re) == v.dirty.get() && !v.bound.full && v.bound.tilesX == (W + 15u) / 16u) return v.bound;
+    rt::launchBoundFull(fullBound, W, rb, re);
+    return fullBound;
   }
   rt::SkyChain sky;
   size_t skyTiles = 0;
diff --git a/raytracedggx_amd/csrc/visibility.hip b/raytracedggx_amd/csrc/visibility.hip
--- a/raytracedggx_amd/csrc/visibility.hip
+++ b/raytracedggx_amd/csrc/visibility.hip
@@ -270,7 +270,16 @@
   }
   v.flags.rows[0] = rb; v.flags.rows[1] = re; v.flags.rasterFrame = c->frameCounter;
   v.cleared.frame = 0u;
-  const uint32_t nt = c->mesh[0].numTris + c->mesh[1].numTris;
+  { BoundInstance inst[2];
+    for (int i = 0; i < 2; ++i) {
+      const MeshDev& m = c->mesh[i];
+      inst[i].worldViewProj = fp.po[i].WorldViewProj; inst[i].projBias = fp.po[i].ProjBias;
+      inst[i].present = m.numTris > 0u; inst[i].known = !m.deforming;
+      for (int k = 0; k < 3; ++k) { inst[i].bmin[k] = m.bmin[k]; inst[i].bmax[k] = m.bmax[k]; }
+    }
+    computeLaunchBound(v.bound, inst, 2, fp.W, fp.H, rb, re);
+    c->visUses = 0u; }
+  const uint32_t nt =c->mesh[0].numTris + c->mesh[1].numTris;
   FrameParams* const dst = c->slotUploaded ? (FrameParams*)nullptr : c->dParams + c->slot;
   c->slotUploaded = true;
   const dim3 grid(nt ? (nt + 4u * RT_RASTER_TPW - 1u) / (4u * RT_RASTER_TPW) : 1u);
```

Measured after the change: 3337 Mrays/s (median of 6 runs). No clear change (+0.9%).
